# CliMA/ClimaSeaIce.jl

Measured on AMD Instinct MI355X. Metric: EVP sub-cycle cell-updates/s, higher is better.
Workload: dtype f64; 1 GPU; evp_subcycle_fplane_periodic_2048x2048_as_1x1_tiles_of_2048x2048_120substeps; substeps=120, mode=fast, halo=4, halo_exchange=none (one tile)

## Files before the change

climaseaice.jl_amd/csrc/evp_fast_math.h:

```cpp
#pragma once
#include "csi_dev.h"

namespace csi {
namespace fm {

#define CSI_EPS64 2.220446049250313e-16

__device__ __forceinline__ double fma_(double a, double b, double c) { return __builtin_fma(a, b, c); }
__device__ __forceinline__ double fmax_(double a, double b) { return __builtin_fmax(a, b); }
__device__ __forceinline__ double fmin_(double a, double b) { return __builtin_fmin(a, b); }
__device__ __forceinline__ double clampd(double x, double lo, double hi) { return x > hi ? hi : (x < lo ? lo : x); }
__device__ __forceinline__ double avg2(double a, double b) { return 0.5 * (a + b); }
__device__ __forceinline__ double avg4(double a, double b, double c, double d) { return 0.25 * ((a + b) + (c + d)); }
__device__ __forceinline__ double sum2(double a, double b) { return a + b; }
__device__ __forceinline__ double quarter(double s_a, double s_b) { return 0.25 * (s_a + s_b); }

__device__ __forceinline__ double rcp(double x) {
    const double r = __builtin_amdgcn_rcp(x);
    return fma_(fma_(-x, r, 1.0), r, r);
}
__device__ __forceinline__ double rsqrt(double x) {
    const double y = __builtin_amdgcn_rsq(x);
    const double g = x * y, h = 0.5 * y;
    const double r = fma_(-h, g, 0.5);
    return fma_(y, r, y);
}
__device__ __forceinline__ void sqrt_rsqrt(double x, double& s, double& rs) {
    const double y = __builtin_amdgcn_rsq(x);
    double g = x * y, h = 0.5 * y;
    const double r = fma_(-h, g, 0.5);
    g = fma_(g, r, g);
    h = fma_(h, r, h);
    const double d = fma_(-g, g, x);
    s = fma_(d, h, g);
    rs = 2.0 * h;
}
__device__ __forceinline__ double sqrt_fast(double x) {
    const double y = __builtin_amdgcn_rsq(x);
    const double g = x * y, h = 0.5 * y;
    const double r = fma_(-h, g, 0.5);
    return fma_(g, r, g);
}

template <bool UNI>
__device__ __forceinline__ void strain_cell(double A, double Bn, double Bs, double Cn, double Cs,
                                            double u_e, double u_w, double v_n, double v_s, double& e11, double& e22) {
    if (UNI) {
        e11 = A * (u_e - u_w);
        e22 = Cn * (v_n - v_s);
    } else {
        e11 = fma_(A, u_e - u_w, fma_(Bn, v_n, -(Bs * v_s)));
        e22 = fma_(Cn, v_n, -(Cs * v_s));
    }
}
template <bool UNI>
__device__ __forceinline__ double strain_corner(double Sn, double Ss, double Sv, double u_n, double u_s, double v_e, double v_w) {
    if (UNI) return fma_(Sv, v_e - v_w, Sn * (u_n - u_s));
    return fma_(Sv, v_e - v_w, fma_(Sn, u_n, -(Ss * u_s)));
}

struct StressConst {
    double em2, Dmin, Dmin2, rDmin, amin, amax, amin2, amax2, ramin, ramax;
    double hk1;
    int pressure_kind;
    double em2_8, Dmin2_16;
};

struct StressOut {
    double s11, s22, s12, alpha, zc2, zf2;
    double xc, rDc;
};

__device__ __forceinline__ StressOut stress_update_r(const StressConst& k, double e11c, double e22c, double e12f,
                                                     double e11f, double e22f, double e12c, double Pc, double Pf,
                                                     double mc, double mf, double rmc, double rmf, double hkc, double hkf,
                                                     double s11, double s22, double s12) {
    StressOut o;
    const double dc = e11c + e22c, df = e11f + e22f;
    const double tc = e11c - e22c, tf = e11f - e22f;
    const double sc2 = fma_(tc, tc, 4.0 * (e12c * e12c));
    const double sf2 = fma_(tf, tf, 4.0 * (e12f * e12f));
    const double xc = fmax_(fma_(dc, dc, sc2 * k.em2), k.Dmin2), xf = fmax_(fma_(df, df, sf2 * k.em2), k.Dmin2);
    const double rDc = rsqrt(xc), rDf = rsqrt(xf);
    const double zc2 = Pc * rDc, zf2 = Pf * rDf;
    const double Pr = (k.pressure_kind == 0) ? Pc * rcp(fma_(k.Dmin, rDc, 1.0)) : Pc;
    const double ec2 = zc2 * k.em2, ef2 = zf2 * k.em2;
    const double bulk = fma_(zc2 * k.hk1, dc, -0.5 * Pr);
    const double s11n = fma_(ec2, e11c, bulk);
    const double s22n = fma_(ec2, e22c, bulk);
    const double s12n = ef2 * e12f;
    const double g2c_raw = zc2 * hkc * rmc, g2f_raw = zf2 * hkf * rmf;
    const double g2c = fmax_(fmin_(g2c_raw, k.amax2), k.amin2);
    const double g2f = fmax_(fmin_(g2f_raw, k.amax2), k.amin2);
    double gc, rgc, gf, rgf;
    sqrt_rsqrt(g2c, gc, rgc);
    sqrt_rsqrt(g2f, gf, rgf);
    const double wc = (mc > 0) ? rgc : 0.0, wf = (mf > 0) ? rgf : 0.0;
    o.s11 = fma_(s11n - s11, wc, s11);
    o.s22 = fma_(s22n - s22, wc, s22);
    o.s12 = fma_(s12n - s12, wf, s12);
    o.alpha = gc;
    o.zc2 = zc2; o.zf2 = zf2; o.xc = xc; o.rDc = rDc;
    return o;
}

__device__ __forceinline__ StressOut stress_update_s(const StressConst& k, double e11c, double e22c, double E12f,
                                                     double S11f, double S22f, double y2, double Pc, double XP,
                                                     double mc, double M4, double rmc, double rM4, double hkc, double hkf4,
                                                     double s11, double s22, double s12) {
    StressOut o;
    const double dc = e11c + e22c, DF = S11f + S22f;
    const double tc = e11c - e22c, TF = S11f - S22f;
    const double sc2 = fma_(tc, tc, y2 * y2);
    const double sf2 = fma_(TF, TF, E12f * E12f);
    const double xc = fmax_(fma_(dc, dc, sc2 * k.em2), k.Dmin2), xf = fmax_(fma_(DF, DF, sf2 * k.em2), k.Dmin2_16);
    const double rDc = rsqrt(xc), rDf = rsqrt(xf);
    const double zc2 = Pc * rDc, zf2 = XP * rDf;
    const double Pr = (k.pressure_kind == 0) ? Pc * rcp(fma_(k.Dmin, rDc, 1.0)) : Pc;
    const double ec2 = zc2 * k.em2, ef2 = zf2 * k.em2_8;
    const double bulk = fma_(zc2 * k.hk1, dc, -0.5 * Pr);
    const double s11n = fma_(ec2, e11c, bulk);
    const double s22n = fma_(ec2, e22c, bulk);
    const double s12n = ef2 * E12f;
    const double g2c_raw = zc2 * hkc * rmc, g2f_raw = zf2 * hkf4 * rM4;
    const double g2c = fmax_(fmin_(g2c_raw, k.amax2), k.amin2);
    const double g2f = fmax_(fmin_(g2f_raw, k.amax2), k.amin2);
    double gc, rgc, gf, rgf;
    sqrt_rsqrt(g2c, gc, rgc);
    sqrt_rsqrt(g2f, gf, rgf);
    const double wc = (mc > 0) ? rgc : 0.0, wf = (M4 > 0) ? rgf : 0.0;
    o.s11 = fma_(s11n - s11, wc, s11);
    o.s22 = fma_(s22n - s22, wc, s22);
    o.s12 = fma_(s12n - s12, wf, s12);
    o.alpha = gc;
    o.zc2 = zc2; o.zf2 = zf2; o.xc = xc; o.rDc = rDc;
    return o;
}

__device__ __forceinline__ StressOut stress_update(const StressConst& k, double e11c, double e22c, double e12f,
                                                   double e11f, double e22f, double e12c, double Pc, double Pf,
                                                   double mc, double mf, double hkc, double hkf,
                                                   double s11, double s22, double s12) {
    return stress_update_r(k, e11c, e22c, e12f, e11f, e22f, e12c, Pc, Pf, mc, mf, rcp(mc), rcp(mf), hkc, hkf, s11, s22, s12);
}

struct VelConst {
    double dt, rdt, fcor, min_mass, min_conc;
    int has_cor;
};

__device__ __forceinline__ void ext_stress(int kind, double tau, double rhoCd, double we, double webar, double w, double wbar,
                                           double& ex, double& im) {
    if (kind == 3) {
        const double d1 = we - w, d2 = webar - wbar;
        const double n2 = fma_(d1, d1, d2 * d2);
        const double n = sqrt_fast(fmax_(n2, 2.2250738585072014e-308));
        im = rhoCd * n;
        ex = im * we;
    } else {
        ex = tau; im = 0.0;
    }
}

__device__ __forceinline__ void ext_stress_rest(double rhoCd, double w, double wbar, double& ex, double& im) {
    const double n2 = fma_(w, w, wbar * wbar);
    im = rhoCd * sqrt_fast(fmax_(n2, 2.2250738585072014e-308));
    ex = 0.0;
}

__device__ __forceinline__ double vel_update_avg(const VelConst& k, double w, double wn, double mi, double ai, double abar,
                                                 double div, double cor, double ext, double imt, double exb, double imb, bool peripheral) {
    const double rm = rcp(mi);
    const double rai = rm * ai;
    const double G = fma_(wn - w, k.rdt, fma_(div, rm, fma_(exb - ext, rai, cor)));
    const double tau_i = (imb - imt) * rai;
    const double wD = fma_(k.dt, G, abar * w) * rcp(fma_(k.dt, tau_i, abar));
    const bool active_ice = (mi >= k.min_mass) & (ai >= k.min_conc);
    double res = active_ice ? wD : 0.0;
    return peripheral ? 0.0 : res;
}
__device__ __forceinline__ double vel_update_avg_fd(const VelConst& k, double w, double wn, double mi, double ai, double abar,
                                                    double div, double cor, double ext, double imt, double exb, double imb,
                                                    bool peripheral, double wf) {
    const double wD = vel_update_avg(k, w, wn, mi, ai, abar, div, cor, ext, imt, exb, imb, false);
    const bool active_ice = (mi >= k.min_mass) & (ai >= k.min_conc);
    const bool marginal = (mi > CSI_EPS64) & (ai > CSI_EPS64);
    const double res = active_ice ? wD : (marginal ? wf : 0.0);
    return peripheral ? 0.0 : res;
}
__device__ __forceinline__ double vel_update(const VelConst& k, double w, double wn, double m_a, double m_b, double a_a, double a_b,
                                             double al_a, double al_b, double div, double cor,
                                             double ext, double imt, double exb, double imb, bool peripheral) {
    return vel_update_avg(k, w, wn, avg2(m_a, m_b), avg2(a_a, a_b), avg2(al_a, al_b), div, cor, ext, imt, exb, imb, peripheral);
}
__device__ __forceinline__ double vel_update_fd(const VelConst& k, double w, double wn, double m_a, double m_b, double a_a, double a_b,
                                                double al_a, double al_b, double div, double cor,
                                                double ext, double imt, double exb, double imb, bool peripheral, double wf) {
    return vel_update_avg_fd(k, w, wn, avg2(m_a, m_b), avg2(a_a, a_b), avg2(al_a, al_b), div, cor, ext, imt, exb, imb, peripheral, wf);
}

__device__ __forceinline__ double vel_update_sum(const VelConst& k2, double w, double wn, double m2, double a2, double al2,
                                                 double div2, double cor, double ext, double imt, double exb, double imb, bool peripheral) {
    const double rm2 = rcp(m2);
    const double rai = rm2 * a2;
    const double G = fma_(wn - w, k2.rdt, fma_(div2, rm2, fma_(exb - ext, rai, cor)));
    const double tau_i = (imb - imt) * rai;
    const double wD = fma_(k2.dt, G, al2 * w) * rcp(fma_(k2.dt, tau_i, al2));
    const bool active_ice = (m2 >= k2.min_mass) & (a2 >= k2.min_conc);
    double res = active_ice ? wD : 0.0;
    return peripheral ? 0.0 : res;
}
__device__ __forceinline__ double vel_update_sum_fd(const VelConst& k2, double w, double wn, double m2, double a2, double al2,
                                                    double div2, double cor, double ext, double imt, double exb, double imb,
                                                    bool peripheral, double wf) {
    const double wD = vel_update_sum(k2, w, wn, m2, a2, al2, div2, cor, ext, imt, exb, imb, false);
    const bool active_ice = (m2 >= k2.min_mass) & (a2 >= k2.min_conc);
    const bool marginal = (m2 > 2.0 * CSI_EPS64) & (a2 > 2.0 * CSI_EPS64);
    const double res = active_ice ? wD : (marginal ? wf : 0.0);
    return peripheral ? 0.0 : res;
}

__device__ __forceinline__ double div1(double E, double Fn, double Fs, double s11_0, double s11_m, double s12_p, double s12_0) {
    return fma_(E, s11_0 - s11_m, fma_(Fn, s12_p, -(Fs * s12_0)));
}
template <bool UNI>
__device__ __forceinline__ double div2(double Q1n, double Q2n, double Q1s, double Q2s, double K,
                                       double s11_0, double s22_0, double s11_m, double s22_m, double s12_p, double s12_0) {
    if (UNI) return fma_(K, s12_p - s12_0, Q2n * (s22_0 - s22_m));
    const double n = fma_(Q1n, s11_0, Q2n * s22_0);
    const double s = fma_(Q1s, s11_m, Q2s * s22_m);
    return fma_(K, s12_p - s12_0, n - s);
}

__device__ __forceinline__ void full_strain_cell(double Uy_e, double Uy_w, double Vx_n, double Vx_s, double Ur_e, double Ur_w,
                                                 double Vr_n, double Vr_s, double dyc2, double dxc2, double razc, double& e11, double& e22) {
    const double D1 = (Uy_e - Uy_w) + (Vx_n - Vx_s);
    const double D2 = fma_(dyc2, Ur_e - Ur_w, -(dxc2 * (Vr_n - Vr_s)));
    const double hr = 0.5 * razc;
    e11 = hr * (D1 + D2);
    e22 = hr * (D1 - D2);
}
__device__ __forceinline__ double full_strain_corner(double Ux_n, double Ux_s, double Vy_e, double Vy_w, double dxf2, double dyf2, double razf) {
    return (0.5 * razf) * fma_(dxf2, Ux_n - Ux_s, dyf2 * (Vy_e - Vy_w));
}
__device__ __forceinline__ double full_div1(double dyu, double rdyu, double rdxu, double razu, double S_e, double S_w, double T_e, double T_w,
                                            double Z_n, double Z_s) {
    return razu * fma_(0.5 * dyu, S_e - S_w, fma_(0.5 * rdyu, T_e - T_w, rdxu * (Z_n - Z_s)));
}
__device__ __forceinline__ double full_div2(double dxv, double rdxv, double rdyv, double razv, double S_n, double S_s, double T_n, double T_s,
                                            double Z_e, double Z_w) {
    return razv * fma_(0.5 * dxv, S_n - S_s, fma_(-0.5 * rdxv, T_n - T_s, rdyv * (Z_e - Z_w)));
}

__device__ __forceinline__ double full_strain_corner8(double Ux_n, double Ux_s, double Vy_e, double Vy_w, double dxf2, double dyf2, double razf) {
    return (4.0 * razf) * fma_(dxf2, Ux_n - Ux_s, dyf2 * (Vy_e - Vy_w));
}
__device__ __forceinline__ double full_div1_x2(double dyu, double rdyu, double rdxu, double razu, double S_e, double S_w, double T_e, double T_w,
                                               double Z_n, double Z_s) {
    return razu * fma_(dyu, S_e - S_w, fma_(rdyu, T_e - T_w, (rdxu + rdxu) * (Z_n - Z_s)));
}
__device__ __forceinline__ double full_div2_x2(double dxv, double rdxv, double rdyv, double razv, double S_n, double S_s, double T_n, double T_s,
                                               double Z_e, double Z_w) {
    return razv * fma_(dxv, S_n - S_s, fma_(-rdxv, T_n - T_s, (rdyv + rdyv) * (Z_e - Z_w)));
}

}
}
```

climaseaice.jl_amd/csrc/evp_fused2.hip:

```cpp
#include "evp_pair_stage.h"

#include <cstdio>
#include <cstdlib>

#ifndef CSI_PAIR_WAVES
#define CSI_PAIR_WAVES 3
#endif
#ifndef CSI_PAIR_UNI_WAVES
#define CSI_PAIR_UNI_WAVES 2
#endif
#ifndef CSI_PAIR_FULL_WAVES
#define CSI_PAIR_FULL_WAVES 2
#endif
#ifndef CSI_PAIR_PRIO
#define CSI_PAIR_PRIO 2
#endif
#ifndef CSI_PAIR_HOIST
#define CSI_PAIR_HOIST 1
#endif
#ifndef CSI_FULL_FENCE
#define CSI_FULL_FENCE 1
#endif
#ifndef CSI_PAIR_STORES
#define CSI_PAIR_STORES 7
#endif
#ifndef CSI_PEER_EXP
#define CSI_PEER_EXP 3
#endif
#ifndef CSI_PAIR_SKIPB
#define CSI_PAIR_SKIPB 0
#endif
#ifndef CSI_PAIR_PD
#define CSI_PAIR_PD 1
#endif

namespace csi {
namespace fused {

#ifdef CSI_PAIR_PROBE
static __device__ unsigned long long g_probe[8192 * 16];
#define PROBE_DECL unsigned long long pacc0 = 0, pacc1 = 0, pacc2 = 0, ptprev = 0, pit = 0; const unsigned long long pwall0 = wall_clock64()
#define PROBE_START do { __builtin_amdgcn_sched_barrier(0); ptprev = __builtin_readcyclecounter(); __builtin_amdgcn_sched_barrier(0); ++pit; } while (0)
#define PROBE(acc) do { __builtin_amdgcn_sched_barrier(0); const unsigned long long t_ = __builtin_readcyclecounter(); \
                        __builtin_amdgcn_sched_barrier(0); acc += t_ - ptprev; ptprev = t_; } while (0)
#define PROBE_END(slot) do { if (lane == 0 && (slot) < 8192 && !write_diag) { unsigned long long* dbg = g_probe + (size_t)(slot) * 16; \
                        dbg[0] = pacc0; dbg[1] = pacc1; dbg[2] = pacc2; dbg[6] = pit; dbg[8] = pwall0; dbg[9] = wall_clock64(); \
                        dbg[12] = PSTAGE.sp0; dbg[13] = PSTAGE.sp1; dbg[14] = PSTAGE.sp2; dbg[15] = PSTAGE.sp3; \
                        dbg[10] = (unsigned long long)__builtin_amdgcn_s_getreg((31 << 11) | (0 << 6) | 4); dbg[11] = (unsigned long long)blockIdx.x; } } while (0)
#else
#define PROBE_DECL do { } while (0)
#define PROBE_START do { } while (0)
#define PROBE(acc) do { } while (0)
#define PROBE_END(slot) do { } while (0)
#endif

template <int V> struct Idx { static constexpr int value = V; };

constexpr int RING_ROWS = 4;
enum : int { RF_S11 = 0, RF_S22, RF_S12, RF_U, RF_V, RF_P, RF_M, RF_A, RF_UN, RF_VN, RF_PF, RF_RMC, RF_RMF };
#ifndef CSI_PAIR_LDSC_NOPRE
#define CSI_PAIR_LDSC_NOPRE 1
#endif
#ifndef CSI_PAIR_PRE
#define CSI_PAIR_PRE 1
#endif
#ifndef CSI_PAIR_FRING
#define CSI_PAIR_FRING 1
#endif
constexpr int RF_FORCING = 8;
enum : int { RF_FU_TAU = 10, RF_FU_WE, RF_FU_WB, RF_FU_FD, RF_FV_TAU, RF_FV_WE, RF_FV_WB, RF_FV_FD };
constexpr int RP_ROWS = 3, RP_FIELDS = 12;
enum : int { RP_DXV = 0, RP_RDYV, RP_RDXU, RP_DXF2, RP_DYF2, RP_RAZF, RP_DYU, RP_DYC2, RP_DXC2, RP_RAZC, RP_RAZU, RP_RAZV };

template <bool UNI, bool AUF, bool WALLS, bool MASK, bool FORCE, bool FD, int CF, bool FULL = false, bool PEER = false, int EXTRA = 0, bool DLD = false>
__device__ __forceinline__ void pair_body(const FusedTable* __restrict__ table, const int w, int nstrips, int nchunks, int rows,
                                       int blocks_per_xcd, int write_diag, unsigned long long seq,
                                       double* __restrict__ ring, unsigned* __restrict__ ringm, double* __restrict__ outr, unsigned* __restrict__ peer_abort_p, double* __restrict__ ringp,
                                       double* __restrict__ ringc) {
    constexpr bool LDSC = !UNI && !FULL && !(EXTRA == 1 && MASK) && (CSI_PAIR_LDSC != 0);
    constexpr bool FRING = FORCE && !FULL && (EXTRA != 1 || !MASK) && CSI_PAIR_FRING;
    constexpr bool PRE = CSI_PAIR_PRE && !MASK && !FULL && !FRING && !(CSI_PAIR_LDSC_NOPRE && !UNI && !(EXTRA == 1 && MASK) && (CSI_PAIR_LDSC != 0));
    constexpr int RING_FIELDS = FRING ? 10 + RF_FORCING : (PRE ? 13 : 10);
#define peer_abort (*peer_abort_p)
    const int b = (int)blockIdx.x;
#ifndef CSI_EXP_ROLESWAP
#define CSI_EXP_ROLESWAP 0
#endif
    const bool consumer = (__builtin_amdgcn_readfirstlane((int)(threadIdx.x >> 6)) != 0) != (CSI_EXP_ROLESWAP && ((((b >> 3) / CSI_EXP_ROLESWAP) & 1) != 0));
    const int chunk = w / nstrips, strip = w - chunk * nstrips;
    const int lane = (int)(threadIdx.x & 63);
    tptr_t T = (tptr_t)table;
    const bool single = (write_diag & 2) != 0;
    write_diag &= 1;

    int ja, jb, rstart, rend;
    unsigned loff, sc, sf;
    unsigned lm = 0, sm = 0;
    int i;
    unsigned flags;
    int dx;
    int dxv;
    bool wave_valx_b = false;
    bool wave_has_dx_b;
    bool lanes_uniform;
    bool lanes_same;
    int row0;
    enum : unsigned { L_RS = 1, L_R1 = 2, L_R2 = 4, L_WALL_U = 8, L_WALL_V = 16, L_MIR_LO = 32, L_MIR_HI = 64, L_VAL_LO = 128, L_VAL_HI = 256, L_LOW = 512 };
    {
        const int Nx = T->I[FI_NX], Hx = T->I[FI_HX], Hy = T->I[FI_HY];
        const int i0s = T->I[FI_DEC + 0] - P_LO + strip * P_W;
        i = i0s + lane;
        {
            const int elo = T->I[FI_ELO] > 0 ? T->I[FI_ELO] : rows;
            ja = (T->I[FI_EHI] > 0 && chunk == nchunks - 1 && chunk > 0) ? T->I[FI_DEC + 3] - T->I[FI_EHI] + 1
                                                                         : T->I[FI_DEC + 2] + (chunk == 0 ? 0 : elo + (chunk - 1) * rows);
            jb = chunk == 0 ? min(ja + elo - 1, T->I[FI_DEC + 3])
                            : (chunk == nchunks - 1 ? T->I[FI_DEC + 3] : min(ja + rows - 1, T->I[FI_DEC + 3] - T->I[FI_EHI]));
        }
        const int ic = min(max(i, 1 - Hx), Nx + Hx);
        loff = (unsigned)(ic - (1 - Hx)) * 8u;
        row0 = 1 - Hy;
        const bool own = (lane >= P_LO) & (lane <= P_HI) & (i <= T->I[FI_DEC + 1]);
        flags = 0;
        if (own & (i >= T->I[FI_RS + 0]) & (i <= T->I[FI_RS + 1])) flags |= L_RS;
        if (own & (i >= T->I[FI_R1 + 0]) & (i <= T->I[FI_R1 + 1])) flags |= L_R1;
        if (own & (i >= T->I[FI_R2 + 0]) & (i <= T->I[FI_R2 + 1])) flags |= L_R2;
        dx = 0;
        if ((T->I[FI_XLO] == SIDE_PERIODIC) & (i >= 1) & (i <= Hx)) dx = Nx * 8;
        else if ((T->I[FI_XHI] == SIDE_PERIODIC) & (i > Nx - Hx) & (i <= Nx)) dx = -Nx * 8;
        dxv = dx;
        if (WALLS) {
            const bool xlo_wall = T->I[FI_XLO] == SIDE_WALL, xhi_wall = T->I[FI_XHI] == SIDE_WALL;
            if ((xlo_wall & (i <= 1)) | (xhi_wall & (i > Nx))) flags |= L_WALL_U;
            if ((xlo_wall & (i < 1)) | (xhi_wall & (i > Nx))) flags |= L_WALL_V;
            if (xlo_wall & (i == 0)) flags |= L_MIR_LO;
            if (xhi_wall & (i == Nx + 1)) flags |= L_MIR_HI;
            const bool vval_lo = T->I[FI_IMV + 0] == IMG_VALUE, vval_hi = T->I[FI_IMV + 1] == IMG_VALUE;
            if (xlo_wall & (i >= 1) & (i <= Hx)) dxv = vval_lo ? ((i == 1) ? -8 : 0) : (1 - 2 * i) * 8;
            if (xhi_wall & (i > Nx - Hx) & (i <= Nx)) dxv = vval_hi ? ((i == Nx) ? 8 : 0) : (2 * Nx + 1 - 2 * i) * 8;
            if (xlo_wall & vval_lo & ((i == 1) | (i == 0))) flags |= L_VAL_LO;
            if (xhi_wall & vval_hi & ((i == Nx) | (i == Nx + 1))) flags |= L_VAL_HI;
            wave_valx_b = __builtin_amdgcn_ballot_w64((flags & (L_VAL_LO | L_VAL_HI)) != 0) != 0;
        }
        wave_has_dx_b = __builtin_amdgcn_ballot_w64((dx != 0) | (dxv != 0)) != 0;
        const bool same = ((flags & L_RS) != 0) == ((flags & L_R1) != 0) && ((flags & L_RS) != 0) == ((flags & L_R2) != 0);
        lanes_same = __builtin_amdgcn_ballot_w64(!same) == 0;
        lanes_uniform = !wave_has_dx_b && lanes_same;
        rstart = max(ja - 3, T->I[FI_AJ0]);
#ifndef CSI_EXP_RINGCUT
#define CSI_EXP_RINGCUT 0
#endif
        rend = min(jb + 3 - CSI_EXP_RINGCUT, T->I[FI_AJ1]);
        if (i <= Hx) flags |= L_LOW;
        sc = (unsigned)T->I[FI_LD_C] * 8u;
        sf = (unsigned)T->I[FI_LD_F] * 8u;
        if (MASK) {
            sm = (unsigned)T->I[FI_MASK_LD];
            lm = (unsigned)(ic - (1 - Hx));
        }
    }
    unsigned pdirs = 0;
    if constexpr (PEER) {
        const bool pw = strip < T->I[FI_PSET], pe = strip >= nstrips - T->I[FI_PSET + 1], ps = chunk < T->I[FI_PSET + 2],
                   pn = chunk >= nchunks - T->I[FI_PSET + 3];
        pdirs = ((pw ? 1u : 0u) | (pe ? 2u : 0u) | (ps ? 4u : 0u) | (pn ? 8u : 0u) | ((ps & pw) ? 16u : 0u) | ((ps & pe) ? 32u : 0u) |
                 ((pn & pw) ? 64u : 0u) | ((pn & pe) ? 128u : 0u)) & (unsigned)T->I[FI_PMASK];
        pdirs = (unsigned)__builtin_amdgcn_readfirstlane((int)pdirs);
        if (pdirs) {
            if (!consumer && !(CSI_PEER_EXP & 4)) {
                const unsigned long long t0 = wall_clock64();
                bool dead = false;
                for (;;) {
                    bool behind = false, poison = false;
                    if constexpr ((CSI_PEER_EXP & 8) != 0) {
                        const unsigned long long* slots = (const unsigned long long*)T->P[FP_SLOT_IN + 2];
                        if (lane < 15) {
                            const int cq = (chunk + lane / 3 - 2 + 2 * nchunks) % nchunks, cs = (strip + lane % 3 - 1 + nstrips) % nstrips;
                            behind |= __hip_atomic_load(slots + (cq * nstrips + cs), __ATOMIC_RELAXED, __HIP_MEMORY_SCOPE_SYSTEM) + 1ull < seq;
                        }
                    } else
#pragma unroll
                    for (int d = 0; d < 8; ++d) {
                        if (!((pdirs >> d) & 1u)) continue;
                        const int nslots = T->I[FI_PWAIT + d];
                        const unsigned long long* slots = (const unsigned long long*)T->P[FP_SLOT_IN + d];
#pragma unroll 1
                        for (int b0 = 0; b0 < nslots; b0 += 64) {
                            const int idx = b0 + lane;
                            if (idx < nslots) behind |= __hip_atomic_load(slots + idx, __ATOMIC_RELAXED, __HIP_MEMORY_SCOPE_SYSTEM) + 1ull < seq;
                        }
                        if (lane == 63) poison |= __hip_atomic_load(slots + (kPeerSlots - 1), __ATOMIC_RELAXED, __HIP_MEMORY_SCOPE_SYSTEM) != 0ull;
                    }
                    if (__builtin_amdgcn_ballot_w64(behind) == 0) break;
                    if (__builtin_amdgcn_ballot_w64(poison | (*(volatile unsigned*)T->P[FP_PERR] != 0u)) != 0 || wall_clock64() - t0 > 300000000ull) { dead = true; break; }
                    __builtin_amdgcn_s_sleep(8);
                }
                if (dead) {
                    if (lane == 0) *(volatile unsigned*)T->P[FP_PERR] = 1u;
                    if (lane < 8) {
                        typedef const __attribute__((address_space(4))) unsigned long* sptr_t;
                        unsigned long long* out = (unsigned long long*)((sptr_t)&T->P[FP_SLOT_OUT])[lane];
                        if (out) __hip_atomic_store(out + (kPeerSlots - 1), 1ull, __ATOMIC_RELAXED, __HIP_MEMORY_SCOPE_SYSTEM);
                    }
                }
                if (lane == 0) peer_abort = dead ? 1u : 0u;
                if (T->I[FI_PTIER] >= 1) __builtin_amdgcn_fence(__ATOMIC_ACQUIRE, "");
                __builtin_amdgcn_sched_barrier(0);
            }
            __syncthreads();
            if (peer_abort) return;
        }
    }
    auto offc = [&](int j) __attribute__((always_inline)) { return loff + (unsigned)(j - row0) * sc; };
    auto offf = [&](int j) __attribute__((always_inline)) { return loff + (unsigned)(j - row0) * sf; };
    auto offm = [&](int j) __attribute__((always_inline)) { return lm + (unsigned)(j - row0) * sm; };
    const int NyW = T->I[FI_NY], HyW = T->I[FI_HY];
    int rcd = 0;
    if constexpr (FULL) {
        typedef const __attribute__((address_space(4))) int* iptr_t;
        iptr_t rcs = (iptr_t)T->P[FP_RCSUM];
        if (rcs) {
            const int t0 = max(rstart - 4, row0) - row0, t1 = min(rend + 2, NyW + HyW + 1) - row0;
            if (rcs[t1 + 1] - rcs[t0] == t1 - t0 + 1) rcd = FP_C2ROW_0 - FP_C2_0;
        }
    }
    const unsigned c2s = FULL ? (rcd ? 8u : (unsigned)T->I[FI_C2_LD] * 8u) : 0u;
    const unsigned loff2 = (FULL && rcd) ? 0u : loff;
    auto off2 = [&](int j) __attribute__((always_inline)) { return loff2 + (unsigned)(j - row0) * c2s; };
    const int NyLoW = PEER ? T->I[FI_NYLO] : NyW;
    const bool wrap_lo_b = T->I[FI_YLO] == SIDE_PERIODIC, wrap_hi_b = T->I[FI_YHI] == SIDE_PERIODIC;
    const bool ylo_wall_b = WALLS && T->I[FI_YLO] == SIDE_WALL, yhi_wall_b = WALLS && T->I[FI_YHI] == SIDE_WALL;
    const bool uval_lo_b = WALLS && T->I[FI_IMU + 2] == IMG_VALUE, uval_hi_b = WALLS && T->I[FI_IMU + 3] == IMG_VALUE;
    enum : unsigned { U_WRAPLO = 1, U_YLO = 2, U_YHI = 4, U_UVLO = 8, U_UVHI = 16, U_HASDX = 32, U_VALX = 64, U_WRAPHI = 128, U_MIR = 256 };
    const bool wave_mir_b = WALLS && __builtin_amdgcn_ballot_w64((flags & (L_MIR_LO | L_MIR_HI)) != 0) != 0;
    const unsigned UF = (unsigned)__builtin_amdgcn_readfirstlane((int)((wrap_lo_b ? U_WRAPLO : 0u) | (wrap_hi_b ? U_WRAPHI : 0u) | (ylo_wall_b ? U_YLO : 0u) | (yhi_wall_b ? U_YHI : 0u) |
                                                                         (uval_lo_b ? U_UVLO : 0u) | (uval_hi_b ? U_UVHI : 0u) |
                                                                         (wave_has_dx_b ? U_HASDX : 0u) | (wave_valx_b ? U_VALX : 0u) | (wave_mir_b ? U_MIR : 0u)));
#define wrap_lo ((UF & U_WRAPLO) != 0)
#define wrap_hi ((UF & U_WRAPHI) != 0)
#define ylo_wall (WALLS && (UF & U_YLO) != 0)
#define yhi_wall (WALLS && (UF & U_YHI) != 0)
#define uval_lo (WALLS && (UF & U_UVLO) != 0)
#define uval_hi (WALLS && (UF & U_UVHI) != 0)
#define wave_has_dx ((UF & U_HASDX) != 0)
#define wave_valx (WALLS && (UF & U_VALX) != 0)
#define wave_mir (WALLS && (UF & U_MIR) != 0)
#define has_dld (PEER && DLD)
    auto wall_row = [&](int j) __attribute__((always_inline)) { return (ylo_wall & (j < 1)) | (yhi_wall & (j > NyW)); };
    auto wall_vrow = [&](int j) __attribute__((always_inline)) { return (ylo_wall & (j <= 1)) | (yhi_wall & (j > NyW)); };
    const bool lane_wu = WALLS && (flags & L_WALL_U) != 0, lane_wv = WALLS && (flags & L_WALL_V) != 0;
    auto numbers = [&](Forcing& F) __attribute__((always_inline)) {
        F.t_tau_u = T->K[FK_TOP_TAU_U]; F.t_we_u = T->K[FK_TOP_UE]; F.t_wb_u = T->K[FK_TOP_VE];
        F.b_tau_u = T->K[FK_BOT_TAU_U]; F.b_we_u = T->K[FK_BOT_UE]; F.b_wb_u = T->K[FK_BOT_VE];
        F.t_tau_v = T->K[FK_TOP_TAU_V]; F.t_we_v = T->K[FK_TOP_VE]; F.t_wb_v = T->K[FK_TOP_UE];
        F.b_tau_v = T->K[FK_BOT_TAU_V]; F.b_we_v = T->K[FK_BOT_VE]; F.b_wb_v = T->K[FK_BOT_UE];
        F.fd_u = 0.0; F.fd_v = 0.0; F.fd = FD;
        F.xc_u = 0.0; F.xd_u = 0.0; F.xc_v = 0.0; F.xd_v = 0.0; F.extra = EXTRA == 1 ? T->I[FI_EXTRA] : 0;
    };
    auto arrays = [&](Forcing& F, unsigned ou, unsigned ov) __attribute__((always_inline)) {
        if (T->I[FI_TOP_KIND] == 2) { F.t_tau_u = ldg(T->P[FP_FT_U], ou); F.t_tau_v = ldg(T->P[FP_FT_V], ov); }
        if constexpr (EXTRA == 2) {
            if (T->I[FI_TOP_UEK] == 2) { F.t_we_u = ldg(T->P[FP_FT_U], ou); F.t_wb_v = ldg(T->P[FP_FT_UBAR], ov); }
            if (T->I[FI_TOP_VEK] == 2) { F.t_we_v = ldg(T->P[FP_FT_V], ov); F.t_wb_u = ldg(T->P[FP_FT_VBAR], ou); }
            if (T->I[FI_BOT_KIND] == 2) { F.b_tau_u = ldg(T->P[FP_FB_U], ou); F.b_tau_v = ldg(T->P[FP_FB_V], ov); }
        }
        if (T->I[FI_BOT_UEK] == 2) { F.b_we_u = ldg(T->P[FP_FB_U], ou); F.b_wb_v = ldg(T->P[FP_FB_UBAR], ov); }
        if (T->I[FI_BOT_VEK] == 2) { F.b_we_v = ldg(T->P[FP_FB_V], ov); F.b_wb_u = ldg(T->P[FP_FB_VBAR], ou); }
        if (FD) { F.fd_u = ldg(T->P[FP_FD_U], ou); F.fd_v = ldg(T->P[FP_FD_V], ov); }
        if (EXTRA == 1) {
            if (F.extra & 1) { F.xc_u = ldg(T->P[FP_XC_U], ou); F.xc_v = ldg(T->P[FP_XC_V], ov); }
            if (F.extra & 2) { F.xd_u = ldg(T->P[FP_XD_U], ou); F.xd_v = ldg(T->P[FP_XD_V], ov); }
        }
    };
    auto stress_consts = [&](fm::StressConst& ks) __attribute__((always_inline)) {
        ks.em2 = T->K[FK_EM2]; ks.Dmin = T->K[FK_DMIN]; ks.Dmin2 = T->K[FK_DMIN2]; ks.rDmin = T->K[FK_RDMIN];
        ks.amin = T->K[FK_AMIN]; ks.amax = T->K[FK_AMAX]; ks.amin2 = T->K[FK_AMIN2]; ks.amax2 = T->K[FK_AMAX2];
        ks.ramin = T->K[FK_RAMIN]; ks.ramax = T->K[FK_RAMAX]; ks.hk1 = T->K[FK_HK1]; ks.pressure_kind = T->I[FI_PRESSURE_KIND];
        ks.em2_8 = T->K[FK_PK_EM2_8]; ks.Dmin2_16 = T->K[FK_PK_DMIN2_16];
    };
    auto vel_consts = [&](fm::VelConst& kv) __attribute__((always_inline)) {
        kv.dt = T->K[FK_DT2]; kv.rdt = T->K[FK_RDT]; kv.fcor = T->K[FK_FCOR]; kv.min_mass = T->K[FK_MIN_MASS2];
        kv.min_conc = T->K[FK_MIN_CONC2]; kv.has_cor = T->I[FI_HAS_COR];
    };
    const int prio_rank = (int)(__builtin_amdgcn_s_getreg((3 << 11) | (0 << 6) | 4) % 3u);
    auto set_prio = [&](int k) __attribute__((always_inline)) {
        if (CSI_PAIR_PRIO == 2) {
            if (consumer) __builtin_amdgcn_s_setprio(2); else __builtin_amdgcn_s_setprio(0);
        } else if (CSI_PAIR_PRIO == 3) {
            if (consumer) __builtin_amdgcn_s_setprio(0); else __builtin_amdgcn_s_setprio(2);
        } else if (CSI_PAIR_PRIO == 4) {
            if (consumer) __builtin_amdgcn_s_setprio(3); else __builtin_amdgcn_s_setprio(0);
        } else if (CSI_PAIR_PRIO) {
            int p = prio_rank + k;
            p = p >= 3 ? p - 3 : p;
            if (p == 0) __builtin_amdgcn_s_setprio(0); else if (p == 1) __builtin_amdgcn_s_setprio(1); else __builtin_amdgcn_s_setprio(2);
        }
    };
    const int rs_lo = max(ja, T->I[FI_RS + 2]), rs_hi = min(jb, T->I[FI_RS + 3]);
    const int r1_lo = max(ja, T->I[FI_R1 + 2]), r1_hi = min(jb, T->I[FI_R1 + 3]);
    const int r2_lo = max(ja, T->I[FI_R2 + 2]), r2_hi = min(jb, T->I[FI_R2 + 3]);
    auto yimg = [&](int j) __attribute__((always_inline)) {
        return (wrap_lo & (j >= 1) & (j <= HyW)) ? NyLoW : ((wrap_hi & (j > NyW - HyW) & (j <= NyW)) ? -NyW : 0);
    };
    auto yimg_u = [&](int j) __attribute__((always_inline)) {
        int d = yimg(j);
        if (WALLS) {
            if (ylo_wall & (j >= 1) & (j <= HyW)) d = uval_lo ? ((j == 1) ? -1 : 0) : 1 - 2 * j;
            if (yhi_wall & (j > NyW - HyW) & (j <= NyW)) d = uval_hi ? ((j == NyW) ? 1 : 0) : 2 * NyW + 1 - 2 * j;
        }
        return d;
    };
    enum : int { D_W = 0, D_E, D_S, D_N, D_SW, D_SE, D_NW, D_NE };
    auto own = [&](int k) __attribute__((always_inline)) { return T->P[k < 5 ? FP_S11_OUT + k : FP_AL + (k - 5)]; };
    auto img = [&](int k, int d) __attribute__((always_inline)) { return PEER ? T->P[FP_IMG0 + d * 9 + k] : own(k); };
    const bool wave_low = PEER && __builtin_amdgcn_ballot_w64(((flags & L_LOW) != 0) & ((dx != 0) | (dxv != 0))) != 0;
    const bool wt = T->I[FI_WT] != 0;
    auto sto = [&](unsigned long b_, unsigned o_, double v_) __attribute__((always_inline)) {
        if (wt) stg_agent(b_, o_, v_); else stg(b_, o_, v_);
    };
    auto put4 = [&](int k, unsigned off, unsigned dy, bool ylow, int dxl, double val, double valy, double valx, double valxy, int j, int yr) __attribute__((always_inline)) {
        const unsigned long base = own(k);
        auto sti = [&](unsigned long b_, unsigned o_, double v_) __attribute__((always_inline)) {
            if constexpr (PEER && (CSI_PEER_EXP & 2) != 0)
                __scoped_atomic_store_n((__attribute__((address_space(1))) long*)((gptr_t)b_ + o_), __builtin_bit_cast(long, v_), __ATOMIC_RELAXED, __MEMORY_SCOPE_SYSTEM);
            else sto(b_, o_, v_);
        };
        sto(base, off, val);
        if constexpr (PEER) {
            if (has_dld) {
                const int cls = (k == 2 || k == 3 || k == 7) ? 1 : 0;
                const int p0 = j + HyW - 1, p1 = p0 + yr;
                const int dY = ylow ? D_S : D_N, dX = wave_low ? D_W : D_E;
                const int dXY = ylow ? (wave_low ? D_SW : D_SE) : (wave_low ? D_NW : D_NE);
                if (dy != 0u) sti(img(k, dY), off + dy + (unsigned)(p1 * T->I[FI_PDLD + dY * 2 + cls]), valy);
                if (wave_has_dx && dxl != 0) {
                    sti(img(k, dX), off + (unsigned)dxl + (unsigned)(p0 * T->I[FI_PDLD + dX * 2 + cls]), valx);
                    if (dy != 0u) sti(img(k, dXY), off + (unsigned)dxl + dy + (unsigned)(p1 * T->I[FI_PDLD + dXY * 2 + cls]), valxy);
                }
                return;
            }
        }
        if (dy != 0u) sti(PEER ? (ylow ? img(k, D_S) : img(k, D_N)) : base, off + dy, valy);
        if (wave_has_dx) {
            if (dxl != 0) {
                sti(PEER ? (wave_low ? img(k, D_W) : img(k, D_E)) : base, off + (unsigned)dxl, valx);
                if (dy != 0u) sti(PEER ? (ylow ? (wave_low ? img(k, D_SW) : img(k, D_SE)) : (wave_low ? img(k, D_NW) : img(k, D_NE))) : base, off + (unsigned)dxl + dy, valxy);
            }
        }
    };
    auto put = [&](int k, unsigned off, unsigned dy, bool ylow, int dxl, double val, int j, int yr) __attribute__((always_inline)) {
        put4(k, off, dy, ylow, dxl, val, val, val, val, j, yr);
    };
    auto put_u = [&](unsigned off, int j, unsigned dy, double val, int yr) __attribute__((always_inline)) {
        double vy = val;
        if (WALLS) {
            if (uval_lo & ylo_wall & (j == 1)) vy = 2 * T->K[FK_BCU] - val;
            if (uval_hi & yhi_wall & (j == NyW)) vy = 2 * T->K[FK_BCU + 1] - val;
        }
        put4(3, off, dy, j <= HyW, dx, val, vy, val, vy, j, yr);
    };
    auto put_v = [&](unsigned off, unsigned dy, bool ylow, double val, int j, int yr) __attribute__((always_inline)) {
        double vx = val;
        if (WALLS && wave_valx) {
            if (flags & L_VAL_LO) vx = 2 * T->K[FK_BCV] - val;
            if (flags & L_VAL_HI) vx = 2 * T->K[FK_BCV + 1] - val;
        }
        put4(4, off, dy, ylow, dxv, val, val, vx, vx, j, yr);
    };
    int fast_lo, fast_hi;
    {
        const int d1 = AUF ? 0 : 1;
        fast_lo = max(rs_lo, max(r1_lo + d1, r2_lo + 1));
        fast_hi = min(rs_hi, min(r1_hi + d1, r2_hi + 1));
        if (wrap_lo | ylo_wall) fast_lo = max(fast_lo, HyW + 2);
        if (wrap_hi | yhi_wall) fast_hi = min(fast_hi, NyW - HyW);
    }
    const bool fast_plain = lanes_uniform;
    auto flush = [&](int q, double v11, double v22, double v12, double vfirst, double vsecond, auto WH, auto VFT) __attribute__((always_inline)) {
        constexpr int which = decltype(WH)::value;
        constexpr bool VF = decltype(VFT)::value != 0;
        if (which == 0) return;
        if ((q >= fast_lo) & (q <= fast_hi)) {
            const unsigned ocq = offc(q), ofq = offf(q);
            if (fast_plain) {
                if (flags & L_RS) {
                    if (which & 1) { sto(T->P[FP_S11_OUT], ocq, v11); sto(T->P[FP_S22_OUT], ocq, v22); sto(T->P[FP_S12_OUT], ofq, v12); }
                    if (which & 2) sto(T->P[VF ? FP_V_OUTP : FP_U_OUTP], VF ? ocq : ofq - sf, vfirst);
                    if (which & 4) sto(T->P[VF ? FP_U_OUTP : FP_V_OUTP], VF ? ofq - sf : ocq - sc, vsecond);
                }
            } else {
                const bool ls = (flags & L_RS) != 0, l1 = (flags & L_R1) != 0, l2 = (flags & L_R2) != 0;
                if ((which & 1) && ls) { put(0, ocq, 0u, false, dx, v11, q, 0); put(1, ocq, 0u, false, dx, v22, q, 0); put(2, ofq, 0u, false, dx, v12, q, 0); }
                if (VF) { if ((which & 2) && l1) put_v(ocq, 0u, false, vfirst, q, 0); if ((which & 4) && l2) put(3, ofq - sf, 0u, false, dx, vsecond, q - 1, 0); }
                else { if ((which & 2) && l1) put(3, ofq - sf, 0u, false, dx, vfirst, q - 1, 0); if ((which & 4) && l2) put_v(ocq - sc, 0u, false, vsecond, q - 1, 0); }
            }
            return;
        }
        const int j1 = VF ? q : q - 1, j2 = q - 1;
        const bool do_s = ((which & 1) != 0) & (q >= rs_lo) & (q <= rs_hi), do_1 = ((which & 2) != 0) & (j1 >= r1_lo) & (j1 <= r1_hi),
                   do_2 = ((which & 4) != 0) & (j2 >= r2_lo) & (j2 <= r2_hi);
        if (!(do_s | do_1 | do_2)) return;
        const unsigned ocq = offc(q), ofq = offf(q);
        const unsigned o1 = VF ? ocq : ofq - sf;
        const unsigned o2 = VF ? ofq - sf : ocq - sc;
        const int yq = yimg(q), y1 = VF ? yimg(j1) : yimg_u(j1), y2 = VF ? yimg_u(j2) : yimg(j2);
        if (do_s & ((flags & L_RS) != 0)) {
            put(0, ocq, (unsigned)yq * sc, q <= HyW, dx, v11, q, yq);
            put(1, ocq, (unsigned)yq * sc, q <= HyW, dx, v22, q, yq);
            put(2, ofq, (unsigned)yq * sf, q <= HyW, dx, v12, q, yq);
        }
        if (do_1 & ((flags & L_R1) != 0)) {
            if (VF) put_v(o1, (unsigned)y1 * sc, j1 <= HyW, vfirst, j1, y1); else put_u(o1, j1, (unsigned)y1 * sf, vfirst, y1);
        }
        if (do_2 & ((flags & L_R2) != 0)) {
            if (VF) put_u(o2, j2, (unsigned)y2 * sf, vsecond, y2); else put_v(o2, (unsigned)y2 * sc, j2 <= HyW, vsecond, j2, y2);
        }
    };
    unsigned lane_it = (unsigned)lane;
    auto fresh_lane = [&]() __attribute__((always_inline)) {
        if constexpr (MASK && !FULL) {
            unsigned l;
            asm volatile("v_mbcnt_lo_u32_b32 %0, -1, 0\n\tv_mbcnt_hi_u32_b32 %0, -1, %0" : "=v"(l));
            lane_it = l;
        }
    };
    auto rslot = [&](int j) __attribute__((always_inline)) { return (unsigned)((j - rstart) & (RING_ROWS - 1)) * (RING_FIELDS * 64) + lane_it; };

#ifndef CSI_PAIR_UNROLL
#define CSI_PAIR_UNROLL 3
#endif

    if (!consumer) {
        PROBE_DECL;
        Stage<UNI, AUF, MASK, FORCE, CF, FULL, !(EXTRA == 1 && MASK)> A;
        A.lc = ringc;
        const int cjmin = LDSC ? T->I[FI_COEF_JMIN] : 0, cjmax = LDSC ? T->I[FI_COEF_JMAX] : 0;
        const unsigned ck_lane = (unsigned)min(lane, FC_COUNT - 1) * 8u;
        auto coef_row_base = [&](int j) __attribute__((always_inline)) {
            return T->P[FP_PCOEF_VEC] + (unsigned long)((long)min(max(j, cjmin), cjmax) * (long)(FC_COUNT * 8));
        };
#ifndef CSI_EXP_RINGALIAS
#define CSI_EXP_RINGALIAS 0
#endif
        auto alias_row = [&](int j) __attribute__((always_inline)) { return CSI_EXP_RINGALIAS ? min(max(j, ja + 1), max(jb - 1, ja + 1)) : j; };
        unsigned oc = offc(alias_row(rstart)), of = offf(alias_row(rstart)), om = MASK ? offm(rstart) : 0u;
        {
            const double rho0 = T->K[FK_RHO];
            A.u_m = ldg(T->P[FP_U_IN], of - sf); A.v_m = ldg(T->P[FP_V_IN], oc - sc);
            A.u_0 = ldg(T->P[FP_U_IN], of); A.v_0 = ldg(T->P[FP_V_IN], oc);
            A.a_mm = 0.0; A.a_m = ldg(T->P[FP_A], oc - sc);
            A.m_mm = 0.0; A.m_m = ldg(T->P[FP_H], oc - sc) * rho0 * A.a_m;
            const double P_m = ldg(T->P[FP_P], oc - sc);
            A.XP_m = fm::sum2(from_left(P_m), P_m);
            A.Xm_m = fm::sum2(from_left(A.m_m), A.m_m);
            A.Xa_m = fm::sum2(from_left(A.a_m), A.a_m);
            A.Xv_m = fm::sum2(from_left(A.v_m), A.v_m);
            A.Xv_0 = fm::sum2(from_left(A.v_0), A.v_0);
            double e11_m, e22_m;
            const int jm = rstart - 1;
            A.hoist_uniform(T);
            if constexpr (FULL) {
                const unsigned om2 = off2(jm), o02 = off2(rstart);
                full_cell(T, om2, c2s, A.u_m, A.v_m, A.v_0, e11_m, e22_m, rcd);
                A.e12_0 = 8.0 * full_corner(T, o02, c2s, A.u_0, A.u_m, A.v_0, rcd);
                A.hoist_planes(T, rcd);
                A.full_init(T, o02, om2, c2s);
            } else {
            fm::strain_cell<UNI>(pcoef<UNI>(T, FC_A, jm), pcoef<UNI>(T, FC_BN, jm), pcoef<UNI>(T, FC_BS, jm), pcoef<UNI>(T, FC_CN, jm),
                            pcoef<UNI>(T, FC_CS, jm), from_right(A.u_m), A.u_m, A.v_0, A.v_m, e11_m, e22_m);
            A.e12_0 = fm::strain_corner<UNI>(pcoef<UNI>(T, FC_SN, rstart), pcoef<UNI>(T, FC_SS, rstart), pcoef<UNI>(T, FC_SV, rstart), A.u_0, A.u_m, A.v_0, from_left(A.v_0));
            }
            A.Xe11_m = fm::sum2(from_left(e11_m), e11_m);
            A.Xe22_m = fm::sum2(from_left(e22_m), e22_m);
            A.Ye12_0 = fm::sum2(A.e12_0, from_right(A.e12_0));
            A.XAL_m = 0; A.XS11L_m = 0; A.XS22L_m = 0; A.XW = 0; A.Wprev = 0;
            A.S11_mm = 0; A.S22_mm = 0; A.S12_mm = 0; A.AL_mm = 0; A.S11_m = 0; A.S22_m = 0; A.S12_m = 0; A.AL_m = 0;
            A.S11_0 = 0; A.S22_0 = 0; A.S12_0 = 0; A.AL_0 = 0; A.first = 0; A.second = 0;
        }
#pragma unroll
        for (int q = 0; q < RING_ROWS * RING_FIELDS; ++q) ring[q * 64 + lane] = 0.0;
        if constexpr (FULL) {
#pragma unroll
            for (int q = 0; q < RP_ROWS * RP_FIELDS; ++q) ringp[q * 64 + lane] = 1.0;
            A.RAZU_m = 1.0; A.RAZV_x = 1.0; A.RAZC_0 = 1.0;
        }
        unsigned mhist = 0xffffffffu;
        if (MASK) {
            const bool wi = lane_wv | wall_row(rstart - 1);
            const unsigned act = ldub(T->P[FP_MASK], om - sm);
            mhist = (mhist << 2) | (wi ? 3u : (act ? 0u : 1u));
            ringm[(unsigned)((-1) & (RING_ROWS - 1)) * 64 + (unsigned)lane] = mhist & 3u;
        }
        RowIn R[3];
#ifndef CSI_FULL_HOISTP
#define CSI_FULL_HOISTP 1
#endif
#ifndef CSI_FORCE_HOIST
#define CSI_FORCE_HOIST 0
#endif
        constexpr bool HIN = (FULL && CSI_FULL_HOISTP >= 2) || (FORCE && !FULL && (CSI_FORCE_HOIST & 1));
        const unsigned long hU = HIN ? T->P[FP_U_IN] : 0ul, hV = HIN ? T->P[FP_V_IN] : 0ul, hP = HIN ? T->P[FP_P] : 0ul, hH = HIN ? T->P[FP_H] : 0ul,
                            hA = HIN ? T->P[FP_A] : 0ul, h11 = HIN ? T->P[FP_S11_IN] : 0ul, h22 = HIN ? T->P[FP_S22_IN] : 0ul, h12 = HIN ? T->P[FP_S12_IN] : 0ul,
                            hUN = HIN ? T->P[FP_UN] : 0ul, hVN = HIN ? T->P[FP_VN] : 0ul;
        int rnext = rstart;
        auto load_row = [&](RowIn& Q) __attribute__((always_inline)) {
            if constexpr (HIN) {
                Q.u_p = ldg(hU, of + sf); Q.v_p = ldg(hV, oc + sc);
                Q.P_0 = ldg(hP, oc); Q.h_0 = ldg(hH, oc); Q.a_0 = ldg(hA, oc);
                Q.s11 = ldg(h11, oc); Q.s22 = ldg(h22, oc); Q.s12 = ldg(h12, of);
                Q.un_m = ldg(hUN, of - sf); Q.vn_x = ldg(hVN, AUF ? oc - sc : oc);
            } else {
            Q.u_p = ldg(T->P[FP_U_IN], of + sf); Q.v_p = ldg(T->P[FP_V_IN], oc + sc);
            Q.P_0 = ldg(T->P[FP_P], oc); Q.h_0 = ldg(T->P[FP_H], oc); Q.a_0 = ldg(T->P[FP_A], oc);
            Q.s11 = ldg(T->P[FP_S11_IN], oc); Q.s22 = ldg(T->P[FP_S22_IN], oc); Q.s12 = ldg(T->P[FP_S12_IN], of);
            Q.un_m = ldg(T->P[FP_UN], of - sf); Q.vn_x = ldg(T->P[FP_VN], AUF ? oc - sc : oc);
            }
            Q.mk = MASK ? ldub(T->P[FP_MASK], om) : 1u;
            if constexpr (LDSC) Q.ck = ldg(coef_row_base(rnext + 2), ck_lane);
        };
        auto advance = [&]() __attribute__((always_inline)) {
            const bool more = rnext < rend;
            if (CSI_EXP_RINGALIAS) { rnext += more ? 1 : 0; oc = offc(alias_row(rnext)); of = offf(alias_row(rnext)); return; }
            oc += more ? sc : 0u; of += more ? sf : 0u;
            if (MASK) om += more ? sm : 0u;
            rnext += more ? 1 : 0;
        };
        int r = rstart;
        auto body = [&](auto KK) __attribute__((always_inline)) {
            constexpr int k = decltype(KK)::value;
            if (!CSI_PAIR_HOIST || FORCE || (FULL && CSI_FULL_FENCE)) asm volatile("" : "+s"(T));
            set_prio(k);
            fresh_lane();
            PROBE_START;
            if (CSI_PAIR_PD == 1) __builtin_amdgcn_s_waitcnt(0x0F70);
            else if (MASK) __builtin_amdgcn_s_waitcnt(0x0F70 | 11);
            else __builtin_amdgcn_s_waitcnt(0x0F70 | 10);
            PROBE(pacc0);
            const RowIn& C = R[k];
            if constexpr (LDSC) { if (lane < FC_COUNT) ringc[(unsigned)((r + 2) & 7) * FC_COUNT + (unsigned)lane] = C.ck; }
            const unsigned so = (unsigned)((r - rstart) & 1) * (5 * 64) + (unsigned)lane;
            constexpr int PW = 7 & ~CSI_PAIR_STORES;
            double o11 = 0, o22 = 0, o12 = 0, ofirst = 0, osecond = 0;
            if (PW & 1) { o11 = outr[so]; o22 = outr[so + 64]; o12 = outr[so + 128]; }
            if (PW & 2) ofirst = outr[so + 192];
            if (PW & 4) osecond = outr[so + 256];
            Forcing FA;
            numbers(FA);
            if (FORCE) arrays(FA, offf(r - 1), AUF ? offc(r - 1) : offc(r));
            if constexpr (!FULL) {
                advance();
                load_row(R[(k + CSI_PAIR_PD) % 3]);
            }
            flush(r - 4, o11, o22, o12, ofirst, osecond, Idx<PW>{}, Idx<AUF ? 1 : 0>{});
            fm::StressConst ks; stress_consts(ks);
            fm::VelConst kv; vel_consts(kv);
            const double m_0 = C.h_0 * T->K[FK_RHO] * C.a_0;
            const bool pa1 = WALLS && (AUF ? (lane_wu | wall_row(r - 1)) : (lane_wv | wall_vrow(r)));
            const bool pa2 = WALLS && (AUF ? (lane_wv | wall_vrow(r - 1)) : (lane_wu | wall_row(r - 1)));
            if (MASK) {
                const bool wi = lane_wv | wall_row(r);
                mhist = (mhist << 2) | (wi ? 3u : (C.mk ? 0u : 1u));
            }
            if constexpr (FULL) {
                static_assert(CSI_PAIR_PD == 1, "the per-point-metric producer prefetches one row ahead");
                auto mid = [&]() __attribute__((always_inline)) { advance(); load_row(R[(k + 1) % 3]); };
                A.template step<false>(T, ks, kv, r, C.u_p, C.v_p, C.P_0, m_0, C.a_0, C.s11, C.s22, C.s12, C.un_m, C.vn_x, true, r > rstart, pa1, pa2, mhist, FA,
                                       off2(r), c2s, off2(min(r + 1, rend)), off2(max(r - 1, row0)), mid);
            } else
            A.step(T, ks, kv, r, C.u_p, C.v_p, C.P_0, m_0, C.a_0, C.s11, C.s22, C.s12, C.un_m, C.vn_x, true, r > rstart, pa1, pa2, mhist, FA);
            {
                const unsigned s0 = rslot(r), s1 = rslot(r - 1);
                ring[s0 + RF_S11 * 64] = A.S11_0; ring[s0 + RF_S22 * 64] = A.S22_0; ring[s0 + RF_S12 * 64] = A.S12_0;
                if (AUF) { ring[s1 + RF_U * 64] = A.first; ring[s1 + RF_V * 64] = A.second; }
                else { ring[s0 + RF_V * 64] = A.first; ring[s1 + RF_U * 64] = A.second; }
                if (single) {
                    ring[s0 + RF_P * 64] = A.AL_0; ring[s0 + RF_M * 64] = 0.5 * A.zf; ring[s0 + RF_A * 64] = 0.5 * A.zc; ring[s0 + RF_VN * 64] = A.Dc * A.rDc;
                } else {
                ring[s0 + RF_P * 64] = C.P_0; ring[s0 + RF_M * 64] = m_0; ring[s0 + RF_A * 64] = C.a_0;
                if (PRE) { ring[s0 + RF_PF * 64] = A.Pf_0; ring[s0 + RF_RMC * 64] = A.rmc_0; ring[s0 + RF_RMF * 64] = A.rmf_0; }
                ring[s1 + RF_UN * 64] = C.un_m; ring[(AUF ? s1 : s0) + RF_VN * 64] = C.vn_x;
                }
                if constexpr (FRING) {
                    if constexpr (EXTRA == 2) {
                        const bool tt = T->I[FI_TOP_KIND] == 2, bt = T->I[FI_BOT_KIND] == 2;
                        ring[s0 + RF_FU_TAU * 64] = tt ? FA.t_tau_u : FA.t_we_u; ring[s0 + RF_FU_FD * 64] = FA.t_wb_u;
                        ring[s0 + RF_FU_WE * 64] = bt ? FA.b_tau_u : FA.b_we_u; ring[s0 + RF_FU_WB * 64] = FA.b_wb_u;
                        ring[s0 + RF_FV_TAU * 64] = tt ? FA.t_tau_v : FA.t_we_v; ring[s0 + RF_FV_FD * 64] = FA.t_wb_v;
                        ring[s0 + RF_FV_WE * 64] = bt ? FA.b_tau_v : FA.b_we_v; ring[s0 + RF_FV_WB * 64] = FA.b_wb_v;
                    } else {
                    ring[s0 + RF_FU_TAU * 64] = FA.t_tau_u; ring[s0 + RF_FU_WE * 64] = FA.b_we_u; ring[s0 + RF_FU_WB * 64] = FA.b_wb_u; ring[s0 + RF_FU_FD * 64] = EXTRA == 1 ? FA.xc_u : FA.fd_u;
                    ring[s0 + RF_FV_TAU * 64] = FA.t_tau_v; ring[s0 + RF_FV_WE * 64] = FA.b_we_v; ring[s0 + RF_FV_WB * 64] = FA.b_wb_v; ring[s0 + RF_FV_FD * 64] = EXTRA == 1 ? FA.xc_v : FA.fd_v;
                    }
                }
                if constexpr (FULL) {
                    const unsigned p0 = (unsigned)k * (RP_FIELDS * 64) + lane_it;
                    ringp[p0 + RP_DXV * 64] = A.DXV_p; ringp[p0 + RP_RDYV * 64] = A.RDYV_p; ringp[p0 + RP_RDXU * 64] = A.RDXU_p;
                    ringp[p0 + RP_DXF2 * 64] = A.DXF2_p; ringp[p0 + RP_DYF2 * 64] = A.DYF2_p; ringp[p0 + RP_RAZF * 64] = A.RAZF_p;
                    ringp[p0 + RP_DYU * 64] = A.DYU_0; ringp[p0 + RP_DYC2 * 64] = A.DYC2_0; ringp[p0 + RP_DXC2 * 64] = A.DXC2_0;
                    ringp[p0 + RP_RAZC * 64] = A.RAZC_0; ringp[p0 + RP_RAZU * 64] = A.RAZU_m; ringp[p0 + RP_RAZV * 64] = A.RAZV_x;
                }
                if (MASK) ringm[(unsigned)((r - rstart) & (RING_ROWS - 1)) * 64 + lane_it] = mhist & 3u;
            }
            A.shift(C.u_p, C.v_p, m_0, C.a_0);
            PROBE(pacc1);
#ifndef CSI_EXP_HALFBARRIER
#define CSI_EXP_HALFBARRIER 0
#endif
            if (!(CSI_EXP_HALFBARRIER && ((r - rstart) & 1)))
            __syncthreads();
            PROBE(pacc2);
        };
        if constexpr (LDSC) {
#pragma unroll
            for (int d = -3; d <= 1; ++d) {
                const double v = ldg(coef_row_base(rstart + d), ck_lane);
                if (lane < FC_COUNT) ringc[(unsigned)((rstart + d) & 7) * FC_COUNT + (unsigned)lane] = v;
            }
        }
        load_row(R[0]);
        if (CSI_PAIR_PD == 2) {
            advance();
            load_row(R[1]);
        }
        for (;;) {
            body(Idx<0>{});
            if (++r > rend) break;
            body(Idx<1>{});
            if (++r > rend) break;
            body(Idx<2>{});
            if (++r > rend) break;
        }
        for (int d = 0; d < 2; ++d) {
            const unsigned so = (unsigned)((r - rstart) & 1) * (5 * 64) + (unsigned)lane;
            flush(r - 4, outr[so], outr[so + 64], outr[so + 128], outr[so + 192], outr[so + 256], Idx<(7 & ~CSI_PAIR_STORES)>{}, Idx<AUF ? 1 : 0>{});
            if (d == 0) __syncthreads();
            ++r;
        }
#define PSTAGE A
        PROBE_END(w * 2);
#undef PSTAGE
        return;
    }

    auto publish = [&]() __attribute__((always_inline)) {
        if (PEER && pdirs) {
            if ((CSI_PEER_EXP & 1) && T->I[FI_PTIER] < 2) __builtin_amdgcn_s_waitcnt(0x0F70);
            else { __builtin_amdgcn_fence(__ATOMIC_RELEASE, ""); asm volatile("s_waitcnt vmcnt(0)" ::: "memory"); }
            if ((lane < 8) && ((pdirs >> lane) & 1u)) {
                const int nW = T->I[FI_PSET], nE = T->I[FI_PSET + 1], nN = T->I[FI_PSET + 3];
                const bool xw = (lane == D_W) | (lane == D_SW) | (lane == D_NW), xe = (lane == D_E) | (lane == D_SE) | (lane == D_NE);
                const bool yn = (lane == D_N) | (lane == D_NW) | (lane == D_NE);
                const int xs = xe ? strip - (nstrips - nE) : strip, xn = xw ? nW : (xe ? nE : nstrips);
                const int ys = yn ? chunk - (nchunks - nN) : chunk;
                typedef const __attribute__((address_space(4))) unsigned long* sptr_t;
                unsigned long long* out = (unsigned long long*)((sptr_t)&T->P[FP_SLOT_OUT])[lane];
                __hip_atomic_store(out + (ys * xn + xs), seq, __ATOMIC_RELAXED, __HIP_MEMORY_SCOPE_SYSTEM);
            }
        }
    };

    if (single) {
        {
            const int d1 = AUF ? 1 : 0;
            fast_lo = max(rs_lo, max(r1_lo + d1, r2_lo + 1));
            fast_hi = min(rs_hi, min(r1_hi + d1, r2_hi + 1));
            if (wrap_lo | ylo_wall) fast_lo = max(fast_lo, HyW + 2);
            if (wrap_hi | yhi_wall) fast_hi = min(fast_hi, NyW - HyW);
            }
        for (int r = rstart; r <= rend; ++r) {
            __syncthreads();
            const unsigned s0 = rslot(r), s1 = rslot(r - 1);
            const double v11 = ring[s0 + RF_S11 * 64], v22 = ring[s0 + RF_S22 * 64], v12 = ring[s0 + RF_S12 * 64];
            const double vfirst = AUF ? ring[s1 + RF_U * 64] : ring[s0 + RF_V * 64];
            const double vsecond = AUF ? ring[s1 + RF_V * 64] : ring[s1 + RF_U * 64];
            const double dal = ring[s0 + RF_P * 64], dzf = ring[s0 + RF_M * 64], dzc = ring[s0 + RF_A * 64], ddl = ring[s0 + RF_VN * 64];
            flush(r, v11, v22, v12, vfirst, vsecond, Idx<7>{}, Idx<AUF ? 0 : 1>{});
            if (write_diag) {
                if (((flags & L_RS) != 0) & (r >= rs_lo) & (r <= rs_hi)) {
                    const unsigned ocq = offc(r), ofq = offf(r);
                    const int yq = yimg(r);
                    put(5, ocq, (unsigned)yq * sc, r <= HyW, dx, dal, r, yq);
                    put(7, ofq, (unsigned)yq * sf, r <= HyW, dx, dzf, r, yq);
                    put(6, ocq, (unsigned)yq * sc, r <= HyW, dx, dzc, r, yq);
                    put(8, ocq, (unsigned)yq * sc, r <= HyW, dx, ddl, r, yq);
                }
            }
        }
        __syncthreads();
        publish();
        return;
    }

    PROBE_DECL;
    Stage<UNI, !AUF, MASK, FORCE, CF, FULL, !(EXTRA == 1 && MASK)> B;
    B.lc = ringc;
    B.u_m = 0; B.u_0 = 0; B.v_m = 0; B.v_0 = 0; B.Xv_m = 0; B.Xv_0 = 0;
    B.a_mm = 0; B.a_m = 0; B.m_mm = 0; B.m_m = 0;
    B.XP_m = 0; B.Xm_m = 0; B.Xa_m = 0; B.Xe11_m = 0; B.Xe22_m = 0; B.Ye12_0 = 0; B.e12_0 = 0;
    B.XAL_m = 0; B.XS11L_m = 0; B.XS22L_m = 0; B.XW = 0; B.Wprev = 0;
    B.S11_mm = 0; B.S22_mm = 0; B.S12_mm = 0; B.AL_mm = 0; B.S11_m = 0; B.S22_m = 0; B.S12_m = 0; B.AL_m = 0;
    B.S11_0 = 0; B.S22_0 = 0; B.S12_0 = 0; B.AL_0 = 0; B.first = 0; B.second = 0;
    B.zc = 0; B.zf = 0; B.Dc = 0; B.rDc = 0; B.Pf_0 = 0; B.rmc_0 = 0; B.rmf_0 = 0;
    B.hoist_uniform(T);
    if constexpr (FULL) {
        B.hoist_planes(T, rcd);
        B.full_init(T, off2(max(rstart - 2, row0)), off2(max(rstart - 3, row0)), c2s);
        B.full_prefetch_vel(T, off2(max(rstart - 2, row0)), off2(max(rstart - 3, row0)));
    }
    int fq = 0;
    bool fhave = false;
    double f11 = 0, f22 = 0, f12 = 0, ffirst = 0, fsecond = 0;
    const int rlo = rstart - 1;
    unsigned mhistB = 0xffffffffu;
    double vn_delay = 0.0;
    double razv_delay = 1.0;
    double fvd_tau = 0.0, fvd_we = 0.0, fvd_wb = 0.0, fvd_fd = 0.0;
    int r = rstart;
    auto bodyB = [&](auto KK) __attribute__((always_inline)) {
        if (!CSI_PAIR_HOIST || FORCE || (FULL && CSI_FULL_FENCE)) asm volatile("" : "+s"(T));
        set_prio(decltype(KK)::value);
        const int q = r - 2;
        PROBE_START;
        if (!(CSI_EXP_HALFBARRIER && ((r - rstart) & 1)))
        __syncthreads();
        PROBE(pacc0);
        if constexpr (!FULL && CSI_PAIR_SKIPB) { if (q < ja - 3) return; }
        fresh_lane();
        const unsigned s1 = rslot(r - 1), s2 = rslot(r - 2), s3 = rslot(r - 3);
        double bu_p = ring[s1 + RF_U * 64], bv_p = ring[s1 + RF_V * 64];
        const double s11 = ring[s2 + RF_S11 * 64], s22 = ring[s2 + RF_S22 * 64], s12 = ring[s2 + RF_S12 * 64];
        const double bP_0 = ring[s2 + RF_P * 64], bm_0 = ring[s2 + RF_M * 64], ba_0 = ring[s2 + RF_A * 64];
        if (PRE) { B.Pf_0 = ring[s2 + RF_PF * 64]; B.rmc_0 = ring[s2 + RF_RMC * 64]; B.rmf_0 = ring[s2 + RF_RMF * 64]; }
        const double bun = ring[s3 + RF_UN * 64], vn_new = ring[s2 + RF_VN * 64];
        const double bvn = AUF ? vn_new : vn_delay;
        vn_delay = vn_new;
        const unsigned bmk = MASK ? ringm[(unsigned)((r - 2 - rstart) & (RING_ROWS - 1)) * 64 + lane_it] : 0u;
        if constexpr (FULL) {
            if (fhave) flush(fq, f11, f22, f12, ffirst, fsecond, Idx<(CSI_PAIR_STORES & 7)>{}, Idx<AUF ? 1 : 0>{});
        }
        PROBE(pacc1);
        fm::StressConst ks; stress_consts(ks);
        fm::VelConst kv; vel_consts(kv);
        if (WALLS) {
            if (wave_mir) {
            const double vl = from_left(bv_p), vr = from_right(bv_p);
            double ml = vr, mh = vl;
            if (wave_valx) {
                if (flags & L_VAL_LO) ml = 2 * T->K[FK_BCV] - vr;
                if (flags & L_VAL_HI) mh = 2 * T->K[FK_BCV + 1] - vl;
            }
            bv_p = (flags & L_MIR_LO) ? ml : ((flags & L_MIR_HI) ? mh : bv_p);
            }
            if (ylo_wall & (q == 0)) B.u_0 = uval_lo ? 2 * T->K[FK_BCU] - bu_p : bu_p;
            if (yhi_wall & (q == NyW)) bu_p = uval_hi ? 2 * T->K[FK_BCU + 1] - B.u_0 : B.u_0;
        }
        if (MASK) mhistB = (mhistB << 2) | ((q >= rlo) ? bmk : 3u);
        Forcing FB;
        numbers(FB);
        if constexpr (FRING) {
            const double u0 = ring[s2 + RF_FU_TAU * 64], u1 = ring[s2 + RF_FU_WE * 64], u2 = ring[s2 + RF_FU_WB * 64], u3 = ring[s2 + RF_FU_FD * 64];
            double v0, v1, v2, v3;
            if (AUF) {
                v0 = ring[s1 + RF_FV_TAU * 64]; v1 = ring[s1 + RF_FV_WE * 64]; v2 = ring[s1 + RF_FV_WB * 64]; v3 = ring[s1 + RF_FV_FD * 64];
            } else {
                const double n0 = ring[s2 + RF_FV_TAU * 64], n1 = ring[s2 + RF_FV_WE * 64], n2 = ring[s2 + RF_FV_WB * 64], n3 = ring[s2 + RF_FV_FD * 64];
                v0 = fvd_tau; v1 = fvd_we; v2 = fvd_wb; v3 = fvd_fd;
                fvd_tau = n0; fvd_we = n1; fvd_wb = n2; fvd_fd = n3;
            }
            if constexpr (EXTRA == 2) {
                if (T->I[FI_TOP_KIND] == 2) { FB.t_tau_u = u0; FB.t_tau_v = v0; } else { FB.t_we_u = u0; FB.t_we_v = v0; }
                FB.t_wb_u = u3; FB.t_wb_v = v3;
                if (T->I[FI_BOT_KIND] == 2) { FB.b_tau_u = u1; FB.b_tau_v = v1; } else { FB.b_we_u = u1; FB.b_we_v = v1; }
                FB.b_wb_u = u2; FB.b_wb_v = v2;
            } else {
                FB.t_tau_u = u0; FB.b_we_u = u1; FB.b_wb_u = u2;
                FB.t_tau_v = v0; FB.b_we_v = v1; FB.b_wb_v = v2;
                if (EXTRA == 1) { FB.xc_u = u3; FB.xc_v = v3; } else { FB.fd_u = u3; FB.fd_v = v3; }
            }
        } else if (FORCE) {
            const int qm = max(q - 1, row0), qa = max(q, row0);
#ifndef CSI_EXP_NOCONSLOADS
            arrays(FB, offf(qm), AUF ? offc(qa) : offc(qm));
#endif
        }
        const bool pb1 = WALLS && (!AUF ? (lane_wu | wall_row(q - 1)) : (lane_wv | wall_vrow(q)));
        const bool pb2 = WALLS && (!AUF ? (lane_wv | wall_vrow(q - 1)) : (lane_wu | wall_row(q - 1)));
        if constexpr (FULL) {
            constexpr int kk = decltype(KK)::value;
            auto midB = [&]() __attribute__((always_inline)) {
                const unsigned pn = (unsigned)((kk + 2) % 3) * (RP_FIELDS * 64) + lane_it;
                B.N_DXV = ringp[pn + RP_DXV * 64]; B.N_RDYV = ringp[pn + RP_RDYV * 64]; B.N_RDXU = ringp[pn + RP_RDXU * 64];
                B.N_DXF2 = ringp[pn + RP_DXF2 * 64]; B.N_DYF2 = ringp[pn + RP_DYF2 * 64]; B.N_RAZF = ringp[pn + RP_RAZF * 64];
                B.N_DYU = ringp[pn + RP_DYU * 64]; B.N_DYC2 = ringp[pn + RP_DYC2 * 64]; B.N_DXC2 = ringp[pn + RP_DXC2 * 64];
                B.N_RAZC = ringp[pn + RP_RAZC * 64]; B.N_RAZU = ringp[pn + RP_RAZU * 64];
                if (AUF) B.N_RAZV = ringp[(unsigned)kk * (RP_FIELDS * 64) + lane_it + RP_RAZV * 64];
                else { const double x = ringp[pn + RP_RAZV * 64]; B.N_RAZV = razv_delay; razv_delay = x; }
            };
            B.template step<PRE, decltype(midB), true, true>(T, ks, kv, q, bu_p, bv_p, bP_0, bm_0, ba_0, s11, s22, s12, bun, bvn, q >= ja - 1, q >= ja, pb1, pb2, mhistB, FB,
                   off2(max(q, row0)), c2s, off2(max(q + 1, row0)), off2(max(q - 1, row0)), midB, off2(max(q, row0)));
            fq = q; f11 = B.S11_0; f22 = B.S22_0; f12 = B.S12_0; ffirst = B.first; fsecond = B.second; fhave = true;
        } else {
        B.template step<PRE>(T, ks, kv, q, bu_p, bv_p, bP_0, bm_0, ba_0, s11, s22, s12, bun, bvn, q >= ja - 1, q >= ja, pb1, pb2, mhistB, FB);
        flush(q, B.S11_0, B.S22_0, B.S12_0, B.first, B.second, Idx<(CSI_PAIR_STORES & 7)>{}, Idx<AUF ? 1 : 0>{});
        }
        if ((CSI_PAIR_STORES & 7) != 7) {
            const unsigned so = (unsigned)((r - rstart) & 1) * (5 * 64) + (unsigned)lane;
            if (!(CSI_PAIR_STORES & 1)) { outr[so] = B.S11_0; outr[so + 64] = B.S22_0; outr[so + 128] = B.S12_0; }
            if (!(CSI_PAIR_STORES & 2)) outr[so + 192] = B.first;
            if (!(CSI_PAIR_STORES & 4)) outr[so + 256] = B.second;
        }
        if (write_diag) {
            if (((flags & L_RS) != 0) & (q >= rs_lo) & (q <= rs_hi)) {
                const unsigned ocq = offc(q), ofq = offf(q);
                const int yq = yimg(q);
                put(5, ocq, (unsigned)yq * sc, q <= HyW, dx, B.AL_0, q, yq);
                put(7, ofq, (unsigned)yq * sf, q <= HyW, dx, 0.5 * B.zf, q, yq);
                put(6, ocq, (unsigned)yq * sc, q <= HyW, dx, 0.5 * B.zc, q, yq);
                put(8, ocq, (unsigned)yq * sc, q <= HyW, dx, B.Dc * B.rDc, q, yq);
            }
        }
        B.shift(bu_p, bv_p, bm_0, ba_0);
        PROBE(pacc2);
    };
    for (;;) {
        bodyB(Idx<0>{});
        if (++r > rend) break;
        bodyB(Idx<1>{});
        if (++r > rend) break;
        bodyB(Idx<2>{});
        if (++r > rend) break;
    }
    if constexpr (FULL) {
        if (fhave) flush(fq, f11, f22, f12, ffirst, fsecond, Idx<(CSI_PAIR_STORES & 7)>{}, Idx<AUF ? 1 : 0>{});
    }
    __syncthreads();
    publish();
#define PSTAGE B
    PROBE_END(w * 2 + 1);
#undef PSTAGE
#undef peer_abort
}

template <bool UNI, bool AUF, bool WALLS, bool MASK, bool FORCE, bool FD, int CF, bool FULL = false, bool PEER = false, int EXTRA = 0, bool DLD = false>
__global__ void __launch_bounds__(128, (FULL || (FORCE && (EXTRA != 1 || !MASK) && CSI_PAIR_FRING)) ? CSI_PAIR_FULL_WAVES
                                       : (UNI && !(EXTRA == 1 && MASK)) ? CSI_PAIR_UNI_WAVES : CSI_PAIR_WAVES) k_pair(const FusedTable* __restrict__ table, int nstrips, int nchunks, int rows,
                                                              int blocks_per_xcd, int write_diag, unsigned long long seq) {
    constexpr bool FRING = FORCE && !FULL && (EXTRA != 1 || !MASK) && CSI_PAIR_FRING;
    constexpr bool PRE = CSI_PAIR_PRE && !MASK && !FULL && !FRING && !(CSI_PAIR_LDSC_NOPRE && !UNI && !(EXTRA == 1 && MASK) && (CSI_PAIR_LDSC != 0));
    constexpr int RING_FIELDS = FRING ? 10 + RF_FORCING : (PRE ? 13 : 10);
    __shared__ double ring[RING_ROWS * RING_FIELDS * 64];
    __shared__ double ringp[FULL ? RP_ROWS * RP_FIELDS * 64 : 1];
    __shared__ unsigned ringm[MASK ? RING_ROWS * 64 : 1];
    __shared__ double outr[(CSI_PAIR_STORES & 7) != 7 ? 2 * 5 * 64 : 1];
    __shared__ unsigned peer_abort_w;
#ifdef CSI_EXP_LDSPAD
    __shared__ double lds_pad[(FULL && FORCE) ? CSI_EXP_LDSPAD / 8 : 1];
    if (FULL && FORCE) { lds_pad[threadIdx.x] = 0.0; asm volatile("" :: "v"(lds_pad[threadIdx.x])); }
#endif
    constexpr bool LDSC = !UNI && !FULL && !(EXTRA == 1 && MASK) && (CSI_PAIR_LDSC != 0);
    __shared__ double ringc[LDSC ? 8 * FC_COUNT : 1];
    const int b = (int)blockIdx.x;
    int w = (b & 7) * blocks_per_xcd + (b >> 3);
    if (write_diag & 12) {
        typedef const __attribute__((address_space(4))) int* iptr_t;
        iptr_t act = (iptr_t)((tptr_t)table)->P[(write_diag & 8) ? FP_ACT_LIVE0 : FP_ACT_LIVE];
        const int live = act[0], per = (live + 7) >> 3, k = b >> 3, p = (b & 7) * per + k;
        if ((k >= per) | (p >= live)) return;
        w = act[2 + p];
    } else if (w >= nstrips * nchunks) return;
    if constexpr (PEER) {
        const int chunk = w / nstrips, strip = w - chunk * nstrips;
        tptr_t T = (tptr_t)table;
        const bool pw = strip < T->I[FI_PSET], pe = strip >= nstrips - T->I[FI_PSET + 1], ps = chunk < T->I[FI_PSET + 2],
                   pn = chunk >= nchunks - T->I[FI_PSET + 3];
        const unsigned pd = ((pw ? 1u : 0u) | (pe ? 2u : 0u) | (ps ? 4u : 0u) | (pn ? 8u : 0u) | ((ps & pw) ? 16u : 0u) | ((ps & pe) ? 32u : 0u) |
                             ((pn & pw) ? 64u : 0u) | ((pn & pe) ? 128u : 0u)) & (unsigned)T->I[FI_PMASK];
        if (__builtin_amdgcn_readfirstlane((int)pd) == 0) {
            pair_body<UNI, AUF, WALLS, MASK, FORCE, FD, CF, FULL, false, EXTRA, false>(table, w, nstrips, nchunks, rows, blocks_per_xcd, write_diag, seq, ring, ringm, outr, &peer_abort_w, ringp, ringc);
            return;
        }
    }
    pair_body<UNI, AUF, WALLS, MASK, FORCE, FD, CF, FULL, PEER, EXTRA, DLD>(table, w, nstrips, nchunks, rows, blocks_per_xcd, write_diag, seq, ring, ringm, outr, &peer_abort_w, ringp, ringc);
}

}

#if defined(CSI_PAIR_PROBE) && (!defined(CSI_PAIR_VARIANT) || CSI_PAIR_VARIANT == 0)
extern "C" int csi_debug_probe(unsigned long long* dst) {
    return (int)hipMemcpyFromSymbol(dst, HIP_SYMBOL(fused::g_probe), sizeof(unsigned long long) * 8192 * 16);
}
#endif
#if defined(CSI_PAIR_PROBE) && defined(CSI_PAIR_VARIANT) && CSI_PAIR_VARIANT >= 1
#define CSI_PROBE_NAME_(v) csi_debug_probe_v##v
#define CSI_PROBE_NAME(v) CSI_PROBE_NAME_(v)
extern "C" int CSI_PROBE_NAME(CSI_PAIR_VARIANT)(unsigned long long* dst) {
    return (int)hipMemcpyFromSymbol(dst, HIP_SYMBOL(fused::g_probe), sizeof(unsigned long long) * 8192 * 16);
}
#endif

#ifndef CSI_PAIR_VARIANT
#define CSI_PAIR_VARIANT 0
#endif
#if CSI_PAIR_VARIANT == 0
#define CSI_PAIR_NAME launch_fused_pair_plain
#define CSI_PAIR_FLAGS false, false, false, false
#elif CSI_PAIR_VARIANT == 1
#define CSI_PAIR_NAME launch_fused_pair_walls
#define CSI_PAIR_FLAGS true, false, false, false
#elif CSI_PAIR_VARIANT == 2
#define CSI_PAIR_NAME launch_fused_pair_mask
#define CSI_PAIR_FLAGS true, true, false, false
#elif CSI_PAIR_VARIANT == 3
#define CSI_PAIR_NAME launch_fused_pair_force
#define CSI_PAIR_FLAGS true, false, true, false
#elif CSI_PAIR_VARIANT == 4
#define CSI_PAIR_NAME launch_fused_pair_mask_force
#define CSI_PAIR_FLAGS true, true, true, false
#elif CSI_PAIR_VARIANT == 5
#define CSI_PAIR_NAME launch_fused_pair_force_fd
#define CSI_PAIR_FLAGS true, false, true, true
#elif CSI_PAIR_VARIANT == 6
#define CSI_PAIR_NAME launch_fused_pair_mask_force_fd
#define CSI_PAIR_FLAGS true, true, true, true
#elif CSI_PAIR_VARIANT == 7
#define CSI_PAIR_NAME launch_fused_pair_force_x
#define CSI_PAIR_FLAGS true, false, true, false
#define CSI_PAIR_EXTRA 1
#elif CSI_PAIR_VARIANT == 8
#define CSI_PAIR_NAME launch_fused_pair_mask_force_x
#define CSI_PAIR_FLAGS true, true, true, false
#define CSI_PAIR_EXTRA 1
#elif CSI_PAIR_VARIANT == 9
#define CSI_PAIR_NAME launch_fused_pair_force_w
#define CSI_PAIR_FLAGS true, false, true, false
#define CSI_PAIR_EXTRA 2
#else
#define CSI_PAIR_NAME launch_fused_pair_mask_force_w
#define CSI_PAIR_FLAGS true, true, true, false
#define CSI_PAIR_EXTRA 2
#endif
#ifndef CSI_PAIR_EXTRA
#define CSI_PAIR_EXTRA 0
#endif
void CSI_PAIR_NAME(const FusedTable* dev_table, int metric, bool a_ufirst, int common, int nstrips, int nchunks, int rows,
                   int write_diag, unsigned long long seq, hipStream_t s) {
    const int nblocks = nstrips * nchunks;
    const int per_xcd = (nblocks + 7) / 8;
    dim3 grid((unsigned)(per_xcd * 8)), block(128);
    const bool dld = (seq >> 63) != 0;
    seq &= ~(1ull << 63);
    (void)dld;
#if CSI_PAIR_VARIANT >= 1
#define CSI_LAUNCH_PAIR_(U, A, C, F) do { if (seq && dld) hipLaunchKernelGGL((fused::k_pair<U, A, CSI_PAIR_FLAGS, C, F, true, CSI_PAIR_EXTRA, true>), grid, block, 0, s, dev_table, nstrips, nchunks, rows, per_xcd, write_diag, seq); \
                                          else if (seq) hipLaunchKernelGGL((fused::k_pair<U, A, CSI_PAIR_FLAGS, C, F, true, CSI_PAIR_EXTRA>), grid, block, 0, s, dev_table, nstrips, nchunks, rows, per_xcd, write_diag, seq); \
                                          else hipLaunchKernelGGL((fused::k_pair<U, A, CSI_PAIR_FLAGS, C, F, false, CSI_PAIR_EXTRA>), grid, block, 0, s, dev_table, nstrips, nchunks, rows, per_xcd, write_diag, seq); } while (0)
#else
#define CSI_LAUNCH_PAIR_(U, A, C, F) do { if (seq) hipLaunchKernelGGL((fused::k_pair<U, A, CSI_PAIR_FLAGS, C, F, true, CSI_PAIR_EXTRA>), grid, block, 0, s, dev_table, nstrips, nchunks, rows, per_xcd, write_diag, seq); \
                                          else hipLaunchKernelGGL((fused::k_pair<U, A, CSI_PAIR_FLAGS, C, F, false, CSI_PAIR_EXTRA>), grid, block, 0, s, dev_table, nstrips, nchunks, rows, per_xcd, write_diag, seq); } while (0)
#endif
#if CSI_PAIR_VARIANT <= 2
#define CSI_LAUNCH_PAIR(U, A) do { if (common == 2) CSI_LAUNCH_PAIR_(U, A, 2, false); else if (common) CSI_LAUNCH_PAIR_(U, A, 1, false); else CSI_LAUNCH_PAIR_(U, A, 0, false); } while (0)
#else
#define CSI_LAUNCH_PAIR(U, A) do { (void)common; CSI_LAUNCH_PAIR_(U, A, 0, false); } while (0)
#endif
    if (metric == 2) {
#if CSI_PAIR_VARIANT >= 1 && CSI_PAIR_VARIANT <= 2
        if (common == 2) { if (a_ufirst) CSI_LAUNCH_PAIR_(false, true, 2, true); else CSI_LAUNCH_PAIR_(false, false, 2, true); }
        else { if (a_ufirst) CSI_LAUNCH_PAIR_(false, true, 0, true); else CSI_LAUNCH_PAIR_(false, false, 0, true); }
#elif CSI_PAIR_VARIANT >= 1
        if (a_ufirst) CSI_LAUNCH_PAIR_(false, true, 0, true); else CSI_LAUNCH_PAIR_(false, false, 0, true);
#endif
    } else if (metric == 0) { if (a_ufirst) CSI_LAUNCH_PAIR(true, true); else CSI_LAUNCH_PAIR(true, false); }
    else { if (a_ufirst) CSI_LAUNCH_PAIR(false, true); else CSI_LAUNCH_PAIR(false, false); }
#undef CSI_LAUNCH_PAIR
#undef CSI_LAUNCH_PAIR_
}

#if CSI_PAIR_VARIANT == 0
void launch_fused_pair_walls(const FusedTable*, int, bool, int, int, int, int, int, unsigned long long, hipStream_t);
void launch_fused_pair_mask(const FusedTable*, int, bool, int, int, int, int, int, unsigned long long, hipStream_t);
void launch_fused_pair_force(const FusedTable*, int, bool, int, int, int, int, int, unsigned long long, hipStream_t);
void launch_fused_pair_mask_force(const FusedTable*, int, bool, int, int, int, int, int, unsigned long long, hipStream_t);
void launch_fused_pair_force_fd(const FusedTable*, int, bool, int, int, int, int, int, unsigned long long, hipStream_t);
void launch_fused_pair_mask_force_fd(const FusedTable*, int, bool, int, int, int, int, int, unsigned long long, hipStream_t);
void launch_fused_pair_force_x(const FusedTable*, int, bool, int, int, int, int, int, unsigned long long, hipStream_t);
void launch_fused_pair_mask_force_x(const FusedTable*, int, bool, int, int, int, int, int, unsigned long long, hipStream_t);
void launch_fused_pair_force_w(const FusedTable*, int, bool, int, int, int, int, int, unsigned long long, hipStream_t);
void launch_fused_pair_mask_force_w(const FusedTable*, int, bool, int, int, int, int, int, unsigned long long, hipStream_t);
void launch_fused_pair(const FusedTable* dev_table, int metric, bool a_ufirst, bool walls, bool mask, bool force, bool free_drift, int extra,
                       int common, int nstrips, int nchunks, int rows, int write_diag, unsigned long long seq, hipStream_t s) {
    if (metric == 2) walls = true;
    if (extra == 2 && mask) launch_fused_pair_mask_force_w(dev_table, metric, a_ufirst, common, nstrips, nchunks, rows, write_diag, seq, s);
    else if (extra == 2) launch_fused_pair_force_w(dev_table, metric, a_ufirst, common, nstrips, nchunks, rows, write_diag, seq, s);
    else if (extra && mask) launch_fused_pair_mask_force_x(dev_table, metric, a_ufirst, common, nstrips, nchunks, rows, write_diag, seq, s);
    else if (extra) launch_fused_pair_force_x(dev_table, metric, a_ufirst, common, nstrips, nchunks, rows, write_diag, seq, s);
    else if (free_drift && mask) launch_fused_pair_mask_force_fd(dev_table, metric, a_ufirst, common, nstrips, nchunks, rows, write_diag, seq, s);
    else if (free_drift) launch_fused_pair_force_fd(dev_table, metric, a_ufirst, common, nstrips, nchunks, rows, write_diag, seq, s);
    else if (force && mask) launch_fused_pair_mask_force(dev_table, metric, a_ufirst, common, nstrips, nchunks, rows, write_diag, seq, s);
    else if (force) launch_fused_pair_force(dev_table, metric, a_ufirst, common, nstrips, nchunks, rows, write_diag, seq, s);
    else if (mask) launch_fused_pair_mask(dev_table, metric, a_ufirst, common, nstrips, nchunks, rows, write_diag, seq, s);
    else if (walls) launch_fused_pair_walls(dev_table, metric, a_ufirst, common, nstrips, nchunks, rows, write_diag, seq, s);
    else launch_fused_pair_plain(dev_table, metric, a_ufirst, common, nstrips, nchunks, rows, write_diag, seq, s);
}
#endif

}
```

climaseaice.jl_amd/csrc/evp_pair_stage.h:

```cpp
#pragma once
#include "evp_fused_common.h"

namespace csi {
namespace fused {

constexpr int P_LO = 4, P_HI = 59, P_W = P_HI - P_LO + 1;

struct Forcing {
    double t_tau_u, t_we_u, t_wb_u, b_tau_u, b_we_u, b_wb_u, t_tau_v, t_we_v, t_wb_v, b_tau_v, b_we_v, b_wb_v;
    double fd_u, fd_v;
    bool fd;
    double xc_u, xd_u, xc_v, xd_v;
    int extra;
};

struct RowIn { double u_p, v_p, P_0, h_0, a_0, s11, s22, s12, un_m, vn_x; unsigned mk; double ck; };

__device__ __forceinline__ unsigned left_bits(unsigned x) { return (unsigned)__builtin_amdgcn_mov_dpp((int)x, 0x138, 0xf, 0xf, true); }

__device__ __forceinline__ void full_cell(tptr_t T, unsigned o, unsigned s2, double u_0, double v_0, double v_p, double& e11, double& e22, int rcd = 0) {
    const double dyu = c2at(T, C2_DYU + rcd, o), dxv_s = c2at(T, C2_DXV + rcd, o), dxv_n = c2at(T, C2_DXV + rcd, o + s2);
    const double Uy_w = dyu * u_0, Ur_w = fm::rcp(dyu) * u_0;
    const double Vx_s = dxv_s * v_0, Vr_s = fm::rcp(dxv_s) * v_0;
    const double Vx_n = dxv_n * v_p, Vr_n = fm::rcp(dxv_n) * v_p;
    fm::full_strain_cell(from_right(Uy_w), Uy_w, Vx_n, Vx_s, from_right(Ur_w), Ur_w, Vr_n, Vr_s,
                         c2at(T, C2_DYC2 + rcd, o), c2at(T, C2_DXC2 + rcd, o), c2at(T, C2_RAZC + rcd, o), e11, e22);
}
__device__ __forceinline__ double full_corner(tptr_t T, unsigned o, unsigned s2, double u_n, double u_s, double v_e, int rcd = 0) {
    const double Ux_n = c2at(T, C2_RDXU + rcd, o) * u_n, Ux_s = c2at(T, C2_RDXU + rcd, o - s2) * u_s;
    const double Vy_e = c2at(T, C2_RDYV + rcd, o) * v_e;
    return fm::full_strain_corner(Ux_n, Ux_s, Vy_e, from_left(Vy_e), c2at(T, C2_DXF2 + rcd, o), c2at(T, C2_DYF2 + rcd, o), c2at(T, C2_RAZF + rcd, o));
}

template <bool UNI, bool UFIRST, bool MASK, bool TIGHT = false, int CF = 0, bool FULL = false, bool HOLDK = true>
struct Stage {
    double u_m, u_0, v_m, v_0, Xv_m, Xv_0;
    double a_mm, a_m, m_mm, m_m;
    double XP_m, Xm_m, Xa_m, Xe11_m, Xe22_m, Ye12_0, e12_0;
    double XAL_m, XS11L_m, XW, Wprev;
    double XS22L_m;
    double DXV_0, RDXV_0, RDYV_0, RDXU_0, DXF2_0, DYF2_0, RAZF_0;
    double DXV_m, RDXV_m, RDYV_m, RDXU_m, DXF2_m, DYF2_m, DYU_m, RDYU_m, DYC2_m, DXC2_m, DXC2_mm;
    double DXV_p, RDXV_p, RDYV_p, RDXU_p, DXF2_p, DYF2_p, RAZF_p, DYU_0, RDYU_0, DYC2_0, DXC2_0;
#ifndef CSI_FULL_HOISTP
#define CSI_FULL_HOISTP 1
#endif
#if CSI_FULL_HOISTP >= 1
    unsigned long c2p[12];
    int rcd_ = 0;
    __device__ __forceinline__ void hoist_planes(tptr_t T, int rcd = 0) {
        rcd_ = rcd;
#pragma unroll
        for (int k = 0; k < 12; ++k) c2p[k] = T->P[FP_C2_0 + k + rcd];
    }
    __device__ __forceinline__ double c2m(tptr_t, int which, unsigned off) const { return ldg_keep(c2p[which], off); }
#else
    int rcd_ = 0;
    __device__ __forceinline__ void hoist_planes(tptr_t, int rcd = 0) { rcd_ = rcd; }
    __device__ __forceinline__ double c2m(tptr_t T, int which, unsigned off) const { return c2at(T, which + rcd_, off); }
#endif
    __device__ __forceinline__ unsigned long f2u(tptr_t T) const { return T->P[FP_F2U + rcd_]; }
    __device__ __forceinline__ unsigned long f2v(tptr_t T) const { return T->P[FP_F2V + rcd_]; }
    double RAZC_0, RAZU_m, RAZV_x, FU_m, FV_x;

#ifndef CSI_PAIR_VK
#define CSI_PAIR_VK 1
#endif
    static constexpr bool VKC = UNI && !FULL && HOLDK && (CSI_PAIR_VK != 0);
    double VK_E, VK_FN, VK_FS, VK_FU, VK_Q2N, VK_K, VK_FV, VK_BRHO;
    __device__ __forceinline__ void hoist_uniform(tptr_t T) {
        if constexpr (VKC) {
            VK_E = T->K[FK_PCOEF0 + FC_E]; VK_FN = T->K[FK_PCOEF0 + FC_FN]; VK_FS = T->K[FK_PCOEF0 + FC_FS]; VK_FU = T->K[FK_PCOEF0 + FC_FU];
            VK_Q2N = T->K[FK_PCOEF0 + FC_Q2N]; VK_K = T->K[FK_PCOEF0 + FC_K]; VK_FV = T->K[FK_PCOEF0 + FC_FV]; VK_BRHO = T->K[FK_BOT_RHOCD];
            asm volatile("" : "+v"(VK_E), "+v"(VK_FN), "+v"(VK_FS), "+v"(VK_FU), "+v"(VK_Q2N), "+v"(VK_K), "+v"(VK_FV), "+v"(VK_BRHO));
        }
    }
#ifndef CSI_PAIR_LDSC
#define CSI_PAIR_LDSC 0
#endif
    static constexpr bool LDSC = !UNI && !FULL && HOLDK && (CSI_PAIR_LDSC != 0);
    const double* lc = nullptr;
    __device__ __forceinline__ double pc(tptr_t T, int which, int j) const {
        if constexpr (LDSC) return lc[(unsigned)(j & 7) * FC_COUNT + which]; else return pcoef<UNI>(T, which, j);
    }
    __device__ __forceinline__ double vk(tptr_t T, int which, int j, double held) const { if constexpr (VKC) return held; else return pc(T, which, j); }
    __device__ __forceinline__ double brho(tptr_t T) const { if constexpr (VKC) return VK_BRHO; else return T->K[FK_BOT_RHOCD]; }

    double N_DXV, N_RDYV, N_RDXU, N_DXF2, N_DYF2, N_RAZF, N_DYU, N_DYC2, N_DXC2, N_RAZC;
    double N_RAZU, N_RAZV, N_FU, N_FV;
    __device__ __forceinline__ void full_prefetch_vel(tptr_t T, unsigned on, unsigned om) {
        N_RAZU = c2m(T, C2_RAZU, om); N_RAZV = c2m(T, C2_RAZV, UFIRST ? om : on);
        N_FU = 0.0; N_FV = 0.0;
        if (T->I[FI_FKIND] == 2) { N_FU = ldg(f2u(T), om); N_FV = ldg(f2v(T), UFIRST ? om : on); }
    }
    __device__ __forceinline__ void full_prefetch_f(tptr_t T, unsigned on, unsigned om) {
        N_FU = 0.0; N_FV = 0.0;
        if (T->I[FI_FKIND] == 2) { N_FU = ldg(f2u(T), om); N_FV = ldg(f2v(T), UFIRST ? om : on); }
    }
    __device__ __forceinline__ void full_prefetch(tptr_t T, unsigned on, unsigned s2) {
        N_DXV = c2m(T, C2_DXV, on + s2); N_RDYV = c2m(T, C2_RDYV, on + s2); N_RDXU = c2m(T, C2_RDXU, on + s2);
        N_DXF2 = c2m(T, C2_DXF2, on + s2); N_DYF2 = c2m(T, C2_DYF2, on + s2); N_RAZF = c2m(T, C2_RAZF, on + s2);
        N_DYU = c2m(T, C2_DYU, on); N_DYC2 = c2m(T, C2_DYC2, on); N_DXC2 = c2m(T, C2_DXC2, on); N_RAZC = c2m(T, C2_RAZC, on);
    }
    __device__ __forceinline__ void full_init(tptr_t T, unsigned o, unsigned om, unsigned s2) {
        full_prefetch(T, o, s2);
        DXV_0 = c2m(T, C2_DXV, o); RDXV_0 = fm::rcp(DXV_0); RDYV_0 = c2m(T, C2_RDYV, o); RDXU_0 = c2m(T, C2_RDXU, o);
        DXF2_0 = c2m(T, C2_DXF2, o); DYF2_0 = c2m(T, C2_DYF2, o); RAZF_0 = c2m(T, C2_RAZF, o);
        DXV_m = DXV_0; RDXV_m = RDXV_0; RDYV_m = RDYV_0; RDXU_m = RDXU_0; DXF2_m = DXF2_0; DYF2_m = DYF2_0;
        DYU_m = c2m(T, C2_DYU, o); RDYU_m = fm::rcp(DYU_m); DYC2_m = c2m(T, C2_DYC2, o); DXC2_m = c2m(T, C2_DXC2, o); DXC2_mm = DXC2_m;
    }
    double S11_mm, S22_mm, S12_mm, AL_mm, S11_m, S22_m, S12_m, AL_m;
#ifdef CSI_PAIR_PROBE
    unsigned long long sp0 = 0, sp1 = 0, sp2 = 0, sp3 = 0, spt = 0;
#define SPROBE_START do { __builtin_amdgcn_sched_barrier(0); spt = __builtin_readcyclecounter(); __builtin_amdgcn_sched_barrier(0); } while (0)
#define SPROBE(acc) do { __builtin_amdgcn_sched_barrier(0); const unsigned long long t_ = __builtin_readcyclecounter(); \
                         __builtin_amdgcn_sched_barrier(0); acc += t_ - spt; spt = t_; } while (0)
#else
#define SPROBE_START do { } while (0)
#define SPROBE(acc) do { } while (0)
#endif
    double S11_0, S22_0, S12_0, AL_0, zc, zf, Dc, rDc, first, second;
    double Xv_p, Xa_0, Xm_0, e12_p, XW_next;
    double Pf_0, rmc_0, rmf_0;

    struct NoMid { __device__ __forceinline__ void operator()() const {} };
    template <bool PRE = false, class MID = NoMid, bool ALLPRE = false, bool PLR = false>
    __device__ __forceinline__ void step(tptr_t T, const fm::StressConst& ks_in, const fm::VelConst& kv_in, int r,
                                         double u_p, double v_p, double P_0, double m_0, double a_0,
                                         double s11, double s22, double s12, double un_m, double vn_x,
                                         bool do_stress, bool do_vel, bool per_first, bool per_second, unsigned mh,
                                         const Forcing& F, unsigned o2 = 0u, unsigned s2 = 0u, unsigned o2n = 0u, unsigned o2m = 0u, MID mid = MID(), unsigned o2nm = 0u) {
        SPROBE_START;
        Xa_0 = fm::sum2(from_left(a_0), a_0);
        Xv_p = fm::sum2(from_left(v_p), v_p);
        double e11_0, e22_0;
        if constexpr (FULL) {
            DXV_p = N_DXV; RDXV_p = fm::rcp(DXV_p); RDYV_p = N_RDYV; RDXU_p = N_RDXU;
            DXF2_p = N_DXF2; DYF2_p = N_DYF2; RAZF_p = N_RAZF;
            DYU_0 = N_DYU; RDYU_0 = fm::rcp(DYU_0); DYC2_0 = N_DYC2; DXC2_0 = N_DXC2;
            RAZC_0 = N_RAZC;
            if constexpr (ALLPRE) {
                RAZU_m = N_RAZU; RAZV_x = N_RAZV; FU_m = N_FU; FV_x = N_FV;
            } else if (do_vel) {
                RAZU_m = c2m(T, C2_RAZU, o2m); RAZV_x = c2m(T, C2_RAZV, UFIRST ? o2m : o2);
                if (T->I[FI_FKIND] == 2) { FU_m = ldg(f2u(T), o2m); FV_x = ldg(f2v(T), UFIRST ? o2m : o2); }
            }
            const double Uy_w = DYU_0 * u_0, Ur_w = RDYU_0 * u_0;
            fm::full_strain_cell(from_right(Uy_w), Uy_w, DXV_p * v_p, DXV_0 * v_0, from_right(Ur_w), Ur_w, RDXV_p * v_p, RDXV_0 * v_0,
                                 DYC2_0, DXC2_0, RAZC_0, e11_0, e22_0);
            const double Vy_e = RDYV_p * v_p;
            e12_p = fm::full_strain_corner8(RDXU_p * u_p, RDXU_0 * u_0, Vy_e, from_left(Vy_e), DXF2_p, DYF2_p, RAZF_p);
        } else {
        fm::strain_cell<UNI>(pc(T, FC_A, r), pc(T, FC_BN, r), pc(T, FC_BS, r), pc(T, FC_CN, r),
                        pc(T, FC_CS, r), from_right(u_0), u_0, v_p, v_0, e11_0, e22_0);
        e12_p = fm::strain_corner<UNI>(pc(T, FC_SN, r + 1), pc(T, FC_SS, r + 1), pc(T, FC_SV, r + 1),
                                  u_p, u_0, v_p, from_left(v_p));
        }
        {
            const double Xe11_0 = fm::sum2(from_left(e11_0), e11_0), Xe22_0 = fm::sum2(from_left(e22_0), e22_0);
            const double Ye12_p = fm::sum2(e12_p, from_right(e12_p));
            Xm_0 = fm::sum2(from_left(m_0), m_0);
            const double e11f = fm::sum2(Xe11_m, Xe11_0);
            const double e22f = fm::sum2(Xe22_m, Xe22_0);
            const double e12c = 0.0625 * fm::sum2(Ye12_0, Ye12_p);
            const double mf = fm::sum2(Xm_m, Xm_0);
            if constexpr (!PRE) {
                const double XP_0 = fm::sum2(from_left(P_0), P_0);
                Pf_0 = fm::sum2(XP_m, XP_0);
                XP_m = XP_0;
                rmc_0 = fm::rcp(m_0); rmf_0 = fm::rcp(mf);
            }
            const double Pf = Pf_0;
            Xe11_m = Xe11_0; Xe22_m = Xe22_0; Ye12_0 = Ye12_p;
            SPROBE(sp0);
            if (do_stress) {
                fm::StressConst ks = ks_in;
                if (CF) ks.pressure_kind = 0;
                if (TIGHT) {
                    asm volatile("" : "+s"(T));
                    ks.em2 = T->K[FK_EM2]; ks.Dmin = T->K[FK_DMIN]; ks.Dmin2 = T->K[FK_DMIN2]; ks.amin2 = T->K[FK_AMIN2];
                    ks.amax2 = T->K[FK_AMAX2]; ks.hk1 = T->K[FK_HK1]; ks.pressure_kind = T->I[FI_PRESSURE_KIND];
                    ks.em2_8 = T->K[FK_PK_EM2_8]; ks.Dmin2_16 = T->K[FK_PK_DMIN2_16];
                }
                double kc, kf;
                if constexpr (FULL) { kc = T->K[FK_CA_DT] * RAZC_0; kf = T->K[FK_PK_CA_DT4] * RAZF_0; }
                else { kc = UNI ? T->K[FK_HKC] : T->K[FK_CA_DT] * pc(T, FC_RAZC, r); kf = UNI ? T->K[FK_PK_HKF4] : T->K[FK_PK_CA_DT4] * pc(T, FC_RAZF, r); }
                const fm::StressOut o = fm::stress_update_s(ks, e11_0, e22_0, e12_0, e11f, e22f, e12c, P_0, Pf, m_0, mf, rmc_0, rmf_0, kc, kf, s11, s22, s12);
                S11_0 = o.s11; S22_0 = o.s22; S12_0 = o.s12; AL_0 = o.alpha; zc = o.zc2; zf = o.zf2; Dc = o.xc; rDc = o.rDc;
            }
        }
        double d11_0 = S11_0, d22_0 = S22_0, d12_0 = S12_0, d11_m = S11_m, d22_m = S22_m, d12_m = S12_m, d11_mm = S11_mm, d22_mm = S22_mm;
        double d11_mL = XS11L_m, d22_mL = XS22L_m;
        if (MASK) {
            const unsigned m0 = mh & 3u, m1 = (mh >> 2) & 3u, m2 = (mh >> 4) & 3u;
            const bool pcc_0 = m0 == 1u, pcc_m = m1 == 1u, pcc_mm = m2 == 1u;
            unsigned c0 = m0 | m1, c1 = m1 | m2;
            c0 |= left_bits(c0); c1 |= left_bits(c1);
            const bool pff_0 = (c0 & 3u) == 1u, pff_m = (c1 & 3u) == 1u;
            d11_0 = pcc_0 ? 0.0 : S11_0; d22_0 = pcc_0 ? 0.0 : S22_0;
            d11_m = pcc_m ? 0.0 : S11_m; d22_m = pcc_m ? 0.0 : S22_m;
            d11_mm = pcc_mm ? 0.0 : S11_mm; d22_mm = pcc_mm ? 0.0 : S22_mm;
            d12_0 = pff_0 ? 0.0 : S12_0; d12_m = pff_m ? 0.0 : S12_m;
            d11_mL = from_left(d11_m);
            if constexpr (FULL) d22_mL = from_left(d22_m);
            const bool ia_0 = (m0 & 1u) != 0, ia_m = (m1 & 1u) != 0, ia_mm = (m2 & 1u) != 0;
            const bool ia_mL = (left_bits(m1) & 1u) != 0;
            const bool per_u = ia_m | ia_mL;
            per_first = UFIRST ? per_u : (ia_0 | ia_m);
            per_second = UFIRST ? (ia_m | ia_mm) : per_u;
        }
        auto div1_full = [&]() __attribute__((always_inline)) {
            const double S_e = d11_m + d22_m, T_e = DYC2_m * (d11_m - d22_m);
            const double S_w = MASK ? from_left(S_e) : d11_mL + d22_mL;
            const double T_w = MASK ? from_left(T_e) : from_left(DYC2_m) * (d11_mL - d22_mL);
            return fm::full_div1_x2(DYU_m, RDYU_m, RDXU_m, RAZU_m, S_e, S_w, T_e, T_w, DXF2_0 * d12_0, DXF2_m * d12_m);
        };
        auto div2_full = [&](bool low) __attribute__((always_inline)) {
            if (low) {
                const double Zw = DYF2_m * d12_m;
                return fm::full_div2_x2(DXV_m, RDXV_m, RDYV_m, RAZV_x, d11_m + d22_m, d11_mm + d22_mm,
                                     DXC2_m * (d11_m - d22_m), DXC2_mm * (d11_mm - d22_mm), from_right(Zw), Zw);
            }
            const double Zw = DYF2_0 * d12_0;
            return fm::full_div2_x2(DXV_0, RDXV_0, RDYV_0, RAZV_x, d11_0 + d22_0, d11_m + d22_m,
                                 DXC2_0 * (d11_0 - d22_0), DXC2_m * (d11_m - d22_m), from_right(Zw), Zw);
        };
        auto f_full = [&](int which_row, int which_plane, unsigned o, int j) __attribute__((always_inline)) {
            const int kind = T->I[FI_FKIND];
            if (kind == 2) return which_plane == FP_F2U ? FU_m : FV_x;
            if (kind == 1) { typedef const __attribute__((address_space(4))) double* vptr_t; return ((vptr_t)T->P[which_row])[j]; }
            return T->K[FK_FCOR];
        };
        SPROBE(sp1);
        if constexpr (FULL) {
            __builtin_amdgcn_sched_barrier(0);
            if constexpr (!PLR) full_prefetch(T, o2n, s2);
            if constexpr (ALLPRE) { if constexpr (PLR) full_prefetch_f(T, o2n, o2nm); else full_prefetch_vel(T, o2n, o2nm); }
            mid();
            __builtin_amdgcn_sched_barrier(0);
        }
        SPROBE(sp2);
        fm::VelConst kv = kv_in;
        if (TIGHT) {
            asm volatile("" : "+s"(T));
            kv.dt = T->K[FK_DT2]; kv.rdt = T->K[FK_RDT]; kv.min_mass = T->K[FK_MIN_MASS2]; kv.min_conc = T->K[FK_MIN_CONC2];
        }
        if (!do_vel) {
            XW_next = XW;
        } else if (UFIRST) {
            const int j = r - 1;
            double W_0;
            {
                const double vbar = fm::quarter(Xv_m, Xv_0);
                double div;
                if constexpr (FULL) div = div1_full();
                else div = fm::div1(vk(T, FC_E, j, VK_E), vk(T, FC_FN, j, VK_FN), vk(T, FC_FS, j, VK_FS),
                                            d11_m, d11_mL, d12_0, d12_m);
                double ext, imt, exb, imb;
                if (CF) { ext = F.t_tau_u; imt = 0.0; } else fm::ext_stress(T->I[FI_TOP_KIND], F.t_tau_u, T->K[FK_TOP_RHOCD], F.t_we_u, F.t_wb_u, u_m, vbar, ext, imt);
                if (CF == 2) fm::ext_stress_rest(brho(T), u_m, vbar, exb, imb);
                else fm::ext_stress(CF ? 3 : T->I[FI_BOT_KIND], F.b_tau_u, brho(T), F.b_we_u, F.b_wb_u, u_m, vbar, exb, imb);
                double cor;
                if constexpr (FULL) cor = f_full(FP_FROW_U, FP_F2U, o2 - s2, j) * vbar;
                else cor = vk(T, FC_FU, j, VK_FU) * vbar;
                if (F.extra & 1) cor += F.xc_u;
                if (F.extra & 2) div = fm::fma_(2.0, F.xd_u, div);
                W_0 = F.fd ? fm::vel_update_sum_fd(kv, u_m, un_m, Xm_m, Xa_m, XAL_m, div, cor, ext, imt, exb, imb, per_first, F.fd_u)
                           : fm::vel_update_sum(kv, u_m, un_m, Xm_m, Xa_m, XAL_m, div, cor, ext, imt, exb, imb, per_first);
            }
            const double XW_0 = fm::sum2(W_0, from_right(W_0));
            {
                const double ubar = fm::quarter(XW, XW_0);
                double div;
                if constexpr (FULL) div = div2_full(true);
                else div = fm::div2<UNI>(pc(T, FC_Q1N, j), vk(T, FC_Q2N, j, VK_Q2N), pc(T, FC_Q1S, j),
                                            pc(T, FC_Q2S, j), vk(T, FC_K, j, VK_K),
                                            d11_m, d22_m, d11_mm, d22_mm, from_right(d12_m), d12_m);
                double ext, imt, exb, imb;
                if (CF) { ext = F.t_tau_v; imt = 0.0; } else fm::ext_stress(T->I[FI_TOP_KIND], F.t_tau_v, T->K[FK_TOP_RHOCD], F.t_we_v, F.t_wb_v, v_m, ubar, ext, imt);
                if (CF == 2) fm::ext_stress_rest(brho(T), v_m, ubar, exb, imb);
                else fm::ext_stress(CF ? 3 : T->I[FI_BOT_KIND], F.b_tau_v, brho(T), F.b_we_v, F.b_wb_v, v_m, ubar, exb, imb);
                double cor;
                if constexpr (FULL) cor = -f_full(FP_FROW_V, FP_F2V, o2 - s2, j) * ubar;
                else cor = -vk(T, FC_FV, j, VK_FV) * ubar;
                if (F.extra & 1) cor += F.xc_v;
                if (F.extra & 2) div = fm::fma_(2.0, F.xd_v, div);
                second = F.fd ? fm::vel_update_sum_fd(kv, v_m, vn_x, m_mm + m_m, a_mm + a_m, AL_mm + AL_m, div, cor, ext, imt, exb, imb, per_second, F.fd_v)
                              : fm::vel_update_sum(kv, v_m, vn_x, m_mm + m_m, a_mm + a_m, AL_mm + AL_m, div, cor, ext, imt, exb, imb, per_second);
            }
            first = W_0;
            XW_next = XW_0;
        } else {
            double W_0;
            {
                const double ubar = fm::avg4(u_m, from_right(u_m), u_0, from_right(u_0));
                double div;
                if constexpr (FULL) div = div2_full(false);
                else div = fm::div2<UNI>(pc(T, FC_Q1N, r), vk(T, FC_Q2N, r, VK_Q2N), pc(T, FC_Q1S, r),
                                            pc(T, FC_Q2S, r), vk(T, FC_K, r, VK_K),
                                            d11_0, d22_0, d11_m, d22_m, from_right(d12_0), d12_0);
                double ext, imt, exb, imb;
                if (CF) { ext = F.t_tau_v; imt = 0.0; } else fm::ext_stress(T->I[FI_TOP_KIND], F.t_tau_v, T->K[FK_TOP_RHOCD], F.t_we_v, F.t_wb_v, v_0, ubar, ext, imt);
                if (CF == 2) fm::ext_stress_rest(brho(T), v_0, ubar, exb, imb);
                else fm::ext_stress(CF ? 3 : T->I[FI_BOT_KIND], F.b_tau_v, brho(T), F.b_we_v, F.b_wb_v, v_0, ubar, exb, imb);
                double cor;
                if constexpr (FULL) cor = -f_full(FP_FROW_V, FP_F2V, o2, r) * ubar;
                else cor = -vk(T, FC_FV, r, VK_FV) * ubar;
                if (F.extra & 1) cor += F.xc_v;
                if (F.extra & 2) div = fm::fma_(2.0, F.xd_v, div);
                W_0 = F.fd ? fm::vel_update_sum_fd(kv, v_0, vn_x, m_m + m_0, a_m + a_0, AL_m + AL_0, div, cor, ext, imt, exb, imb, per_first, F.fd_v)
                           : fm::vel_update_sum(kv, v_0, vn_x, m_m + m_0, a_m + a_0, AL_m + AL_0, div, cor, ext, imt, exb, imb, per_first);
            }
            const double XW_0 = fm::sum2(from_left(W_0), W_0);
            {
                const int j = r - 1;
                const double vbar = fm::quarter(XW, XW_0);
                double div;
                if constexpr (FULL) div = div1_full();
                else div = fm::div1(vk(T, FC_E, j, VK_E), vk(T, FC_FN, j, VK_FN), vk(T, FC_FS, j, VK_FS),
                                            d11_m, d11_mL, d12_0, d12_m);
                double ext, imt, exb, imb;
                if (CF) { ext = F.t_tau_u; imt = 0.0; } else fm::ext_stress(T->I[FI_TOP_KIND], F.t_tau_u, T->K[FK_TOP_RHOCD], F.t_we_u, F.t_wb_u, u_m, vbar, ext, imt);
                if (CF == 2) fm::ext_stress_rest(brho(T), u_m, vbar, exb, imb);
                else fm::ext_stress(CF ? 3 : T->I[FI_BOT_KIND], F.b_tau_u, brho(T), F.b_we_u, F.b_wb_u, u_m, vbar, exb, imb);
                double cor;
                if constexpr (FULL) cor = f_full(FP_FROW_U, FP_F2U, o2 - s2, j) * vbar;
                else cor = vk(T, FC_FU, j, VK_FU) * vbar;
                if (F.extra & 1) cor += F.xc_u;
                if (F.extra & 2) div = fm::fma_(2.0, F.xd_u, div);
                second = F.fd ? fm::vel_update_sum_fd(kv, u_m, un_m, Xm_m, Xa_m, XAL_m, div, cor, ext, imt, exb, imb, per_second, F.fd_u)
                              : fm::vel_update_sum(kv, u_m, un_m, Xm_m, Xa_m, XAL_m, div, cor, ext, imt, exb, imb, per_second);
            }
            first = W_0;
            XW_next = XW_0;
        }
        SPROBE(sp3);
    }

    __device__ __forceinline__ void shift(double u_p, double v_p, double m_0, double a_0) {
        u_m = u_0; u_0 = u_p; v_m = v_0; v_0 = v_p;
        Xv_m = Xv_0; Xv_0 = Xv_p;
        a_mm = a_m; a_m = a_0; m_mm = m_m; m_m = m_0;
        Xm_m = Xm_0; Xa_m = Xa_0;
        e12_0 = e12_p;
        S11_mm = S11_m; S22_mm = S22_m; S12_mm = S12_m; AL_mm = AL_m;
        S11_m = S11_0; S22_m = S22_0; S12_m = S12_0; AL_m = AL_0;
        XAL_m = fm::sum2(from_left(AL_0), AL_0); XS11L_m = from_left(S11_0);
        if constexpr (FULL) {
            XS22L_m = from_left(S22_0);
            DXV_m = DXV_0; RDXV_m = RDXV_0; RDYV_m = RDYV_0; RDXU_m = RDXU_0; DXF2_m = DXF2_0; DYF2_m = DYF2_0;
            DXV_0 = DXV_p; RDXV_0 = RDXV_p; RDYV_0 = RDYV_p; RDXU_0 = RDXU_p; DXF2_0 = DXF2_p; DYF2_0 = DYF2_p; RAZF_0 = RAZF_p;
            DYU_m = DYU_0; RDYU_m = RDYU_0; DYC2_m = DYC2_0; DXC2_mm = DXC2_m; DXC2_m = DXC2_0;
        }
        XW = XW_next;
        Wprev = first;
    }
};


}
}
```

Baseline: 71.12 billion cell-updates/s.

## Hand over precomputed mass reciprocals and activity predicates from stage A to stage B

Stage A of the paired EVP pipeline now computes the velocity mass reciprocals, area-over-mass ratios and active/positive-mass predicates, and writes them into the shared-memory ring. Stage B reads these instead of recomputing the reciprocals and comparisons from raw mass and area. This removes duplicate rcp and compare work in stage B. In exchange the ring grows by extra LDS fields plus a predicate word array, which adds LDS traffic and footprint. The change also peels the first two B iterations and cuts the final A iteration with matching barriers, to avoid wasted edge-row work.

```diff
diff --git a/climaseaice.jl_amd/csrc/evp_fast_math.h b/climaseaice.jl_amd/csrc/evp_fast_math.h
--- a/climaseaice.jl_amd/csrc/evp_fast_math.h
+++ b/climaseaice.jl_amd/csrc/evp_fast_math.h
@@ -104,10 +104,11 @@
     return o;
 }
 
-__device__ __forceinline__ StressOut stress_update_s(const StressConst& k, double e11c, double e22c, double E12f,
-                                                     double S11f, double S22f, double y2, double Pc, double XP,
-                                                     double mc, double M4, double rmc, double rM4, double hkc, double hkf4,
-                                                     double s11, double s22, double s12) {
+template <bool PRED>
+__device__ __forceinline__ StressOut stress_update_s_(const StressConst& k, double e11c, double e22c, double E12f,
+                                                      double S11f, double S22f, double y2, double Pc, double XP,
+                                                      double mc, double M4, bool mc_pos, bool M4_pos, double rmc, double rM4, double hkc, double hkf4,
+                                                      double s11, double s22, double s12) {
     StressOut o;
     const double dc = e11c + e22c, DF = S11f + S22f;
     const double tc = e11c - e22c, TF = S11f - S22f;
@@ -128,13 +129,25 @@
     double gc, rgc, gf, rgf;
     sqrt_rsqrt(g2c, gc, rgc);
     sqrt_rsqrt(g2f, gf, rgf);
-    const double wc = (mc > 0) ? rgc : 0.0, wf = (M4 > 0) ? rgf : 0.0;
+    const double wc = (PRED ? mc_pos : (mc > 0)) ? rgc : 0.0, wf = (PRED ? M4_pos : (M4 > 0)) ? rgf : 0.0;
     o.s11 = fma_(s11n - s11, wc, s11);
     o.s22 = fma_(s22n - s22, wc, s22);
     o.s12 = fma_(s12n - s12, wf, s12);
     o.alpha = gc;
     o.zc2 = zc2; o.zf2 = zf2; o.xc = xc; o.rDc = rDc;
     return o;
+}
+__device__ __forceinline__ StressOut stress_update_s(const StressConst& k, double e11c, double e22c, double E12f,
+                                                     double S11f, double S22f, double y2, double Pc, double XP,
+                                                     double mc, double M4, double rmc, double rM4, double hkc, double hkf4,
+                                                     double s11, double s22, double s12) {
+    return stress_update_s_<false>(k, e11c, e22c, E12f, S11f, S22f, y2, Pc, XP, mc, M4, false, false, rmc, rM4, hkc, hkf4, s11, s22, s12);
+}
+__device__ __forceinline__ StressOut stress_update_p(const StressConst& k, double e11c, double e22c, double E12f,
+                                                     double S11f, double S22f, double y2, double Pc, double XP,
+                                                     bool mc_pos, bool M4_pos, double rmc, double rM4, double hkc, double hkf4,
+                                                     double s11, double s22, double s12) {
+    return stress_update_s_<true>(k, e11c, e22c, E12f, S11f, S22f, y2, Pc, XP, 0.0, 0.0, mc_pos, M4_pos, rmc, rM4, hkc, hkf4, s11, s22, s12);
 }
 
 __device__ __forceinline__ StressOut stress_update(const StressConst& k, double e11c, double e22c, double e12f,
@@ -199,6 +212,25 @@
     return vel_update_avg_fd(k, w, wn, avg2(m_a, m_b), avg2(a_a, a_b), avg2(al_a, al_b), div, cor, ext, imt, exb, imb, peripheral, wf);
 }
 
+struct VelMass {
+    double rm2, rai;
+    bool active;
+};
+__device__ __forceinline__ VelMass vel_mass(const VelConst& k2, double m2, double a2) {
+    VelMass h;
+    h.rm2 = rcp(m2);
+    h.rai = h.rm2 * a2;
+    h.active = (m2 >= k2.min_mass) & (a2 >= k2.min_conc);
+    return h;
+}
+__device__ __forceinline__ double vel_update_sum_h(const VelConst& k2, double w, double wn, const VelMass& h, double al2,
+                                                   double div2, double cor, double ext, double imt, double exb, double imb, bool peripheral) {
+    const double G = fma_(wn - w, k2.rdt, fma_(div2, h.rm2, fma_(exb - ext, h.rai, cor)));
+    const double tau_i = (imb - imt) * h.rai;
+    const double wD = fma_(k2.dt, G, al2 * w) * rcp(fma_(k2.dt, tau_i, al2));
+    double res = h.active ? wD : 0.0;
+    return peripheral ? 0.0 : res;
+}
 __device__ __forceinline__ double vel_update_sum(const VelConst& k2, double w, double wn, double m2, double a2, double al2,
                                                  double div2, double cor, double ext, double imt, double exb, double imb, bool peripheral) {
     const double rm2 = rcp(m2);
diff --git a/climaseaice.jl_amd/csrc/evp_fused2.hip b/climaseaice.jl_amd/csrc/evp_fused2.hip
--- a/climaseaice.jl_amd/csrc/evp_fused2.hip
+++ b/climaseaice.jl_amd/csrc/evp_fused2.hip
@@ -29,6 +29,15 @@
 #endif
 #ifndef CSI_PAIR_SKIPB
 #define CSI_PAIR_SKIPB 0
+#endif
+#ifndef CSI_PAIR_PEELB
+#define CSI_PAIR_PEELB 1
+#endif
+#ifndef CSI_PAIR_CUTA
+#define CSI_PAIR_CUTA 1
+#endif
+#ifndef CSI_EXP_HANDREG
+#define CSI_EXP_HANDREG 0
 #endif
 #ifndef CSI_PAIR_PD
 #define CSI_PAIR_PD 1
@@ -64,6 +73,10 @@
 #ifndef CSI_PAIR_PRE
 #define CSI_PAIR_PRE 1
 #endif
+#ifndef CSI_PAIR_HAND
+#define CSI_PAIR_HAND 1
+#endif
+enum : int { RF_HU_RM2 = RF_M, RF_HU_RAI = RF_A, RF_HV_RM2 = 13, RF_HV_RAI = 14 };
 #ifndef CSI_PAIR_FRING
 #define CSI_PAIR_FRING 1
 #endif
@@ -80,7 +93,10 @@
     constexpr bool LDSC = !UNI && !FULL && !(EXTRA == 1 && MASK) && (CSI_PAIR_LDSC != 0);
     constexpr bool FRING = FORCE && !FULL && (EXTRA != 1 || !MASK) && CSI_PAIR_FRING;
     constexpr bool PRE = CSI_PAIR_PRE && !MASK && !FULL && !FRING && !(CSI_PAIR_LDSC_NOPRE && !UNI && !(EXTRA == 1 && MASK) && (CSI_PAIR_LDSC != 0));
-    constexpr int RING_FIELDS = FRING ? 10 + RF_FORCING : (PRE ? 13 : 10);
+    constexpr bool HAND = PRE && UNI && !(EXTRA == 1 && MASK) && CSI_PAIR_HAND;
+    static_assert(!HAND || !FD, "the handed-over velocity terms have no free-drift twin (FD comes with FORCE, which has no PRE)");
+    constexpr int RING_FIELDS = FRING ? 10 + RF_FORCING : (HAND ? 15 : (PRE ? 13 : 10));
+    unsigned* const ringw = ringm;
 #define peer_abort (*peer_abort_p)
     const int b = (int)blockIdx.x;
 #ifndef CSI_EXP_ROLESWAP
@@ -479,6 +495,10 @@
         }
 #pragma unroll
         for (int q = 0; q < RING_ROWS * RING_FIELDS; ++q) ring[q * 64 + lane] = 0.0;
+        if constexpr (HAND) {
+#pragma unroll
+            for (int q = 0; q < RING_ROWS; ++q) ringw[q * 64 + lane] = 0u;
+        }
         if constexpr (FULL) {
 #pragma unroll
             for (int q = 0; q < RP_ROWS * RP_FIELDS; ++q) ringp[q * 64 + lane] = 1.0;
@@ -567,7 +587,7 @@
                 A.template step<false>(T, ks, kv, r, C.u_p, C.v_p, C.P_0, m_0, C.a_0, C.s11, C.s22, C.s12, C.un_m, C.vn_x, true, r > rstart, pa1, pa2, mhist, FA,
                                        off2(r), c2s, off2(min(r + 1, rend)), off2(max(r - 1, row0)), mid);
             } else
-            A.step(T, ks, kv, r, C.u_p, C.v_p, C.P_0, m_0, C.a_0, C.s11, C.s22, C.s12, C.un_m, C.vn_x, true, r > rstart, pa1, pa2, mhist, FA);
+            A.template step<false, typename decltype(A)::NoMid, false, false, HAND && !CSI_EXP_HANDREG>(T, ks, kv, r, C.u_p, C.v_p, C.P_0, m_0, C.a_0, C.s11, C.s22, C.s12, C.un_m, C.vn_x, true, r > rstart, pa1, pa2, mhist, FA);
             {
                 const unsigned s0 = rslot(r), s1 = rslot(r - 1);
                 ring[s0 + RF_S11 * 64] = A.S11_0; ring[s0 + RF_S22 * 64] = A.S22_0; ring[s0 + RF_S12 * 64] = A.S12_0;
@@ -576,7 +596,13 @@
                 if (single) {
                     ring[s0 + RF_P * 64] = A.AL_0; ring[s0 + RF_M * 64] = 0.5 * A.zf; ring[s0 + RF_A * 64] = 0.5 * A.zc; ring[s0 + RF_VN * 64] = A.Dc * A.rDc;
                 } else {
-                ring[s0 + RF_P * 64] = C.P_0; ring[s0 + RF_M * 64] = m_0; ring[s0 + RF_A * 64] = C.a_0;
+                ring[s0 + RF_P * 64] = C.P_0;
+                if constexpr (HAND && CSI_EXP_HANDREG) {
+                } else if constexpr (HAND) {
+                    ring[s0 + RF_HU_RM2 * 64] = A.hu_rm2; ring[s0 + RF_HU_RAI * 64] = A.hu_rai;
+                    ring[s0 + RF_HV_RM2 * 64] = A.hv_rm2; ring[s0 + RF_HV_RAI * 64] = A.hv_rai;
+                    ringw[(unsigned)((r - rstart) & (RING_ROWS - 1)) * 64 + lane_it] = A.h_pred;
+                } else { ring[s0 + RF_M * 64] = m_0; ring[s0 + RF_A * 64] = C.a_0; }
                 if (PRE) { ring[s0 + RF_PF * 64] = A.Pf_0; ring[s0 + RF_RMC * 64] = A.rmc_0; ring[s0 + RF_RMF * 64] = A.rmf_0; }
                 ring[s1 + RF_UN * 64] = C.un_m; ring[(AUF ? s1 : s0) + RF_VN * 64] = C.vn_x;
                 }
@@ -622,14 +648,17 @@
             advance();
             load_row(R[1]);
         }
+        const bool cut_last = CSI_PAIR_CUTA && !AUF && !FULL && !single && rend == jb + 3 && rend > rstart;
+        const int rend_a = cut_last ? rend - 1 : rend;
         for (;;) {
             body(Idx<0>{});
-            if (++r > rend) break;
+            if (++r > rend_a) break;
             body(Idx<1>{});
-            if (++r > rend) break;
+            if (++r > rend_a) break;
             body(Idx<2>{});
-            if (++r > rend) break;
-        }
+            if (++r > rend_a) break;
+        }
+        if (cut_last) { __syncthreads(); ++r; }
         for (int d = 0; d < 2; ++d) {
             const unsigned so = (unsigned)((r - rstart) & 1) * (5 * 64) + (unsigned)lane;
             flush(r - 4, outr[so], outr[so + 64], outr[so + 128], outr[so + 192], outr[so + 256], Idx<(7 & ~CSI_PAIR_STORES)>{}, Idx<AUF ? 1 : 0>{});
@@ -701,6 +730,11 @@
     B.S11_mm = 0; B.S22_mm = 0; B.S12_mm = 0; B.AL_mm = 0; B.S11_m = 0; B.S22_m = 0; B.S12_m = 0; B.AL_m = 0;
     B.S11_0 = 0; B.S22_0 = 0; B.S12_0 = 0; B.AL_0 = 0; B.first = 0; B.second = 0;
     B.zc = 0; B.zf = 0; B.Dc = 0; B.rDc = 0; B.Pf_0 = 0; B.rmc_0 = 0; B.rmf_0 = 0;
+    if constexpr (HAND) { B.hu_rm2 = 0; B.hu_rai = 0; B.hv_rm2 = 0; B.hv_rai = 0; B.h_pred = 0; B.Xa_0 = 0; B.Xm_0 = 0; }
+    if constexpr (HAND && CSI_EXP_HANDREG) {
+        B.hu_rm2 = 1e-3; B.hu_rai = 1e-3; B.hv_rm2 = 1e-3; B.hv_rai = 1e-3; B.h_pred = 15u;
+        asm volatile("" : "+v"(B.hu_rm2), "+v"(B.hu_rai), "+v"(B.hv_rm2), "+v"(B.hv_rai), "+v"(B.h_pred));
+    }
     B.hoist_uniform(T);
     if constexpr (FULL) {
         B.hoist_planes(T, rcd);
@@ -715,6 +749,8 @@
     double vn_delay = 0.0;
     double razv_delay = 1.0;
     double fvd_tau = 0.0, fvd_we = 0.0, fvd_wb = 0.0, fvd_fd = 0.0;
+    double hvd_rm2 = 0.0, hvd_rai = 0.0;
+    unsigned hvd_pred = 0u;
     int r = rstart;
     auto bodyB = [&](auto KK) __attribute__((always_inline)) {
         if (!CSI_PAIR_HOIST || FORCE || (FULL && CSI_FULL_FENCE)) asm volatile("" : "+s"(T));
@@ -729,7 +765,24 @@
         const unsigned s1 = rslot(r - 1), s2 = rslot(r - 2), s3 = rslot(r - 3);
         double bu_p = ring[s1 + RF_U * 64], bv_p = ring[s1 + RF_V * 64];
         const double s11 = ring[s2 + RF_S11 * 64], s22 = ring[s2 + RF_S22 * 64], s12 = ring[s2 + RF_S12 * 64];
-        const double bP_0 = ring[s2 + RF_P * 64], bm_0 = ring[s2 + RF_M * 64], ba_0 = ring[s2 + RF_A * 64];
+        const double bP_0 = ring[s2 + RF_P * 64];
+        double bm_0 = 0.0, ba_0 = 0.0;
+        if constexpr (HAND && CSI_EXP_HANDREG) {
+        } else if constexpr (HAND) {
+            typedef decltype(B) SB;
+            B.hu_rm2 = ring[s2 + RF_HU_RM2 * 64]; B.hu_rai = ring[s2 + RF_HU_RAI * 64];
+            const unsigned pw = ringw[(unsigned)((r - 2 - rstart) & (RING_ROWS - 1)) * 64 + lane_it];
+            if (AUF) {
+                B.hv_rm2 = ring[s1 + RF_HV_RM2 * 64]; B.hv_rai = ring[s1 + RF_HV_RAI * 64];
+                const unsigned pv = ringw[(unsigned)((r - 1 - rstart) & (RING_ROWS - 1)) * 64 + lane_it];
+                B.h_pred = (pw & (SB::HP_MC | SB::HP_M4 | SB::HP_U)) | (pv & SB::HP_V);
+            } else {
+                const double n0 = ring[s2 + RF_HV_RM2 * 64], n1 = ring[s2 + RF_HV_RAI * 64];
+                B.hv_rm2 = hvd_rm2; B.hv_rai = hvd_rai;
+                B.h_pred = (pw & (SB::HP_MC | SB::HP_M4 | SB::HP_U)) | hvd_pred;
+                hvd_rm2 = n0; hvd_rai = n1; hvd_pred = pw & SB::HP_V;
+            }
+        } else { bm_0 = ring[s2 + RF_M * 64]; ba_0 = ring[s2 + RF_A * 64]; }
         if (PRE) { B.Pf_0 = ring[s2 + RF_PF * 64]; B.rmc_0 = ring[s2 + RF_RMC * 64]; B.rmf_0 = ring[s2 + RF_RMF * 64]; }
         const double bun = ring[s3 + RF_UN * 64], vn_new = ring[s2 + RF_VN * 64];
         const double bvn = AUF ? vn_new : vn_delay;
@@ -800,7 +853,7 @@
                    off2(max(q, row0)), c2s, off2(max(q + 1, row0)), off2(max(q - 1, row0)), midB, off2(max(q, row0)));
             fq = q; f11 = B.S11_0; f22 = B.S22_0; f12 = B.S12_0; ffirst = B.first; fsecond = B.second; fhave = true;
         } else {
-        B.template step<PRE>(T, ks, kv, q, bu_p, bv_p, bP_0, bm_0, ba_0, s11, s22, s12, bun, bvn, q >= ja - 1, q >= ja, pb1, pb2, mhistB, FB);
+        B.template step<PRE, typename decltype(B)::NoMid, false, false, HAND>(T, ks, kv, q, bu_p, bv_p, bP_0, bm_0, ba_0, s11, s22, s12, bun, bvn, q >= ja - 1, q >= ja, pb1, pb2, mhistB, FB);
         flush(q, B.S11_0, B.S22_0, B.S12_0, B.first, B.second, Idx<(CSI_PAIR_STORES & 7)>{}, Idx<AUF ? 1 : 0>{});
         }
         if ((CSI_PAIR_STORES & 7) != 7) {
@@ -822,6 +875,9 @@
         B.shift(bu_p, bv_p, bm_0, ba_0);
         PROBE(pacc2);
     };
+    if constexpr (!FULL && !MASK && CSI_PAIR_PEELB && !CSI_PAIR_SKIPB) {
+        if (rstart == ja - 3 && rend >= rstart + 2) { __syncthreads(); __syncthreads(); r += 2; }
+    }
     for (;;) {
         bodyB(Idx<0>{});
         if (++r > rend) break;
@@ -847,10 +903,11 @@
                                                               int blocks_per_xcd, int write_diag, unsigned long long seq) {
     constexpr bool FRING = FORCE && !FULL && (EXTRA != 1 || !MASK) && CSI_PAIR_FRING;
     constexpr bool PRE = CSI_PAIR_PRE && !MASK && !FULL && !FRING && !(CSI_PAIR_LDSC_NOPRE && !UNI && !(EXTRA == 1 && MASK) && (CSI_PAIR_LDSC != 0));
-    constexpr int RING_FIELDS = FRING ? 10 + RF_FORCING : (PRE ? 13 : 10);
+    constexpr bool HAND = PRE && UNI && !(EXTRA == 1 && MASK) && CSI_PAIR_HAND;
+    constexpr int RING_FIELDS = FRING ? 10 + RF_FORCING : (HAND ? 15 : (PRE ? 13 : 10));
     __shared__ double ring[RING_ROWS * RING_FIELDS * 64];
     __shared__ double ringp[FULL ? RP_ROWS * RP_FIELDS * 64 : 1];
-    __shared__ unsigned ringm[MASK ? RING_ROWS * 64 : 1];
+    __shared__ unsigned ringm[(MASK || HAND) ? RING_ROWS * 64 : 1];
     __shared__ double outr[(CSI_PAIR_STORES & 7) != 7 ? 2 * 5 * 64 : 1];
     __shared__ unsigned peer_abort_w;
 #ifdef CSI_EXP_LDSPAD
diff --git a/climaseaice.jl_amd/csrc/evp_pair_stage.h b/climaseaice.jl_amd/csrc/evp_pair_stage.h
--- a/climaseaice.jl_amd/csrc/evp_pair_stage.h
+++ b/climaseaice.jl_amd/csrc/evp_pair_stage.h
@@ -122,16 +122,22 @@
     double S11_0, S22_0, S12_0, AL_0, zc, zf, Dc, rDc, first, second;
     double Xv_p, Xa_0, Xm_0, e12_p, XW_next;
     double Pf_0, rmc_0, rmf_0;
-
+    enum : unsigned { HP_MC = 1, HP_M4 = 2, HP_U = 4, HP_V = 8 };
+    double hu_rm2, hu_rai, hv_rm2, hv_rai;
+    unsigned h_pred;
+
+    struct AtU { static constexpr bool value = true; };
+    struct AtV { static constexpr bool value = false; };
     struct NoMid { __device__ __forceinline__ void operator()() const {} };
-    template <bool PRE = false, class MID = NoMid, bool ALLPRE = false, bool PLR = false>
+    template <bool PRE = false, class MID = NoMid, bool ALLPRE = false, bool PLR = false, bool HAND = false>
     __device__ __forceinline__ void step(tptr_t T, const fm::StressConst& ks_in, const fm::VelConst& kv_in, int r,
                                          double u_p, double v_p, double P_0, double m_0, double a_0,
                                          double s11, double s22, double s12, double un_m, double vn_x,
                                          bool do_stress, bool do_vel, bool per_first, bool per_second, unsigned mh,
                                          const Forcing& F, unsigned o2 = 0u, unsigned s2 = 0u, unsigned o2n = 0u, unsigned o2m = 0u, MID mid = MID(), unsigned o2nm = 0u) {
+        constexpr bool TAKE = HAND && PRE, GIVE = HAND && !PRE;
         SPROBE_START;
-        Xa_0 = fm::sum2(from_left(a_0), a_0);
+        if constexpr (!TAKE) Xa_0 = fm::sum2(from_left(a_0), a_0);
         Xv_p = fm::sum2(from_left(v_p), v_p);
         double e11_0, e22_0;
         if constexpr (FULL) {
@@ -159,11 +165,12 @@
         {
             const double Xe11_0 = fm::sum2(from_left(e11_0), e11_0), Xe22_0 = fm::sum2(from_left(e22_0), e22_0);
             const double Ye12_p = fm::sum2(e12_p, from_right(e12_p));
-            Xm_0 = fm::sum2(from_left(m_0), m_0);
+            if constexpr (!TAKE) Xm_0 = fm::sum2(from_left(m_0), m_0);
             const double e11f = fm::sum2(Xe11_m, Xe11_0);
             const double e22f = fm::sum2(Xe22_m, Xe22_0);
             const double e12c = 0.0625 * fm::sum2(Ye12_0, Ye12_p);
-            const double mf = fm::sum2(Xm_m, Xm_0);
+            double mf = 0.0;
+            if constexpr (!TAKE) mf = fm::sum2(Xm_m, Xm_0);
             if constexpr (!PRE) {
                 const double XP_0 = fm::sum2(from_left(P_0), P_0);
                 Pf_0 = fm::sum2(XP_m, XP_0);
@@ -171,6 +178,7 @@
                 rmc_0 = fm::rcp(m_0); rmf_0 = fm::rcp(mf);
             }
             const double Pf = Pf_0;
+            if constexpr (GIVE) h_pred = ((m_0 > 0) ? (unsigned)HP_MC : 0u) | ((mf > 0) ? (unsigned)HP_M4 : 0u);
             Xe11_m = Xe11_0; Xe22_m = Xe22_0; Ye12_0 = Ye12_p;
             SPROBE(sp0);
             if (do_stress) {
@@ -185,7 +193,8 @@
                 double kc, kf;
                 if constexpr (FULL) { kc = T->K[FK_CA_DT] * RAZC_0; kf = T->K[FK_PK_CA_DT4] * RAZF_0; }
                 else { kc = UNI ? T->K[FK_HKC] : T->K[FK_CA_DT] * pc(T, FC_RAZC, r); kf = UNI ? T->K[FK_PK_HKF4] : T->K[FK_PK_CA_DT4] * pc(T, FC_RAZF, r); }
-                const fm::StressOut o = fm::stress_update_s(ks, e11_0, e22_0, e12_0, e11f, e22f, e12c, P_0, Pf, m_0, mf, rmc_0, rmf_0, kc, kf, s11, s22, s12);
+                const fm::StressOut o = TAKE ? fm::stress_update_p(ks, e11_0, e22_0, e12_0, e11f, e22f, e12c, P_0, Pf, (h_pred & HP_MC) != 0, (h_pred & HP_M4) != 0, rmc_0, rmf_0, kc, kf, s11, s22, s12)
+                                             : fm::stress_update_s(ks, e11_0, e22_0, e12_0, e11f, e22f, e12c, P_0, Pf, m_0, mf, rmc_0, rmf_0, kc, kf, s11, s22, s12);
                 S11_0 = o.s11; S22_0 = o.s22; S12_0 = o.s12; AL_0 = o.alpha; zc = o.zc2; zf = o.zf2; Dc = o.xc; rDc = o.rDc;
             }
         }
@@ -245,6 +254,18 @@
             asm volatile("" : "+s"(T));
             kv.dt = T->K[FK_DT2]; kv.rdt = T->K[FK_RDT]; kv.min_mass = T->K[FK_MIN_MASS2]; kv.min_conc = T->K[FK_MIN_CONC2];
         }
+        fm::VelMass hu = {0.0, 0.0, false}, hv = {0.0, 0.0, false};
+        if constexpr (TAKE) {
+            hu.rm2 = hu_rm2; hu.rai = hu_rai; hu.active = (h_pred & HP_U) != 0;
+            hv.rm2 = hv_rm2; hv.rai = hv_rai; hv.active = (h_pred & HP_V) != 0;
+        } else if constexpr (GIVE) {
+            hu = fm::vel_mass(kv, Xm_m, Xa_m);
+            hv = UFIRST ? fm::vel_mass(kv, m_mm + m_m, a_mm + a_m) : fm::vel_mass(kv, m_m + m_0, a_m + a_0);
+        }
+        auto vupd = [&](auto UF, double w, double wn, double al2, double div, double cor,
+                        double ext, double imt, double exb, double imb, bool per) __attribute__((always_inline)) {
+            return fm::vel_update_sum_h(kv, w, wn, decltype(UF)::value ? hu : hv, al2, div, cor, ext, imt, exb, imb, per);
+        };
         if (!do_vel) {
             XW_next = XW;
         } else if (UFIRST) {
@@ -265,6 +286,8 @@
                 else cor = vk(T, FC_FU, j, VK_FU) * vbar;
                 if (F.extra & 1) cor += F.xc_u;
                 if (F.extra & 2) div = fm::fma_(2.0, F.xd_u, div);
+                if constexpr (HAND) W_0 = vupd(AtU{}, u_m, un_m, XAL_m, div, cor, ext, imt, exb, imb, per_first);
+                else
                 W_0 = F.fd ? fm::vel_update_sum_fd(kv, u_m, un_m, Xm_m, Xa_m, XAL_m, div, cor, ext, imt, exb, imb, per_first, F.fd_u)
                            : fm::vel_update_sum(kv, u_m, un_m, Xm_m, Xa_m, XAL_m, div, cor, ext, imt, exb, imb, per_first);
             }
@@ -285,6 +308,8 @@
                 else cor = -vk(T, FC_FV, j, VK_FV) * ubar;
                 if (F.extra & 1) cor += F.xc_v;
                 if (F.extra & 2) div = fm::fma_(2.0, F.xd_v, div);
+                if constexpr (HAND) second = vupd(AtV{}, v_m, vn_x, AL_mm + AL_m, div, cor, ext, imt, exb, imb, per_second);
+                else
                 second = F.fd ? fm::vel_update_sum_fd(kv, v_m, vn_x, m_mm + m_m, a_mm + a_m, AL_mm + AL_m, div, cor, ext, imt, exb, imb, per_second, F.fd_v)
                               : fm::vel_update_sum(kv, v_m, vn_x, m_mm + m_m, a_mm + a_m, AL_mm + AL_m, div, cor, ext, imt, exb, imb, per_second);
             }
@@ -308,6 +333,8 @@
                 else cor = -vk(T, FC_FV, r, VK_FV) * ubar;
                 if (F.extra & 1) cor += F.xc_v;
                 if (F.extra & 2) div = fm::fma_(2.0, F.xd_v, div);
+                if constexpr (HAND) W_0 = vupd(AtV{}, v_0, vn_x, AL_m + AL_0, div, cor, ext, imt, exb, imb, per_first);
+                else
                 W_0 = F.fd ? fm::vel_update_sum_fd(kv, v_0, vn_x, m_m + m_0, a_m + a_0, AL_m + AL_0, div, cor, ext, imt, exb, imb, per_first, F.fd_v)
                            : fm::vel_update_sum(kv, v_0, vn_x, m_m + m_0, a_m + a_0, AL_m + AL_0, div, cor, ext, imt, exb, imb, per_first);
             }
@@ -328,11 +355,17 @@
                 else cor = vk(T, FC_FU, j, VK_FU) * vbar;
                 if (F.extra & 1) cor += F.xc_u;
                 if (F.extra & 2) div = fm::fma_(2.0, F.xd_u, div);
+                if constexpr (HAND) second = vupd(AtU{}, u_m, un_m, XAL_m, div, cor, ext, imt, exb, imb, per_second);
+                else
                 second = F.fd ? fm::vel_update_sum_fd(kv, u_m, un_m, Xm_m, Xa_m, XAL_m, div, cor, ext, imt, exb, imb, per_second, F.fd_u)
                               : fm::vel_update_sum(kv, u_m, un_m, Xm_m, Xa_m, XAL_m, div, cor, ext, imt, exb, imb, per_second);
             }
             first = W_0;
             XW_next = XW_0;
+        }
+        if constexpr (GIVE) {
+            hu_rm2 = hu.rm2; hu_rai = hu.rai; hv_rm2 = hv.rm2; hv_rai = hv.rai;
+            h_pred |= (hu.active ? (unsigned)HP_U : 0u) | (hv.active ? (unsigned)HP_V : 0u);
         }
         SPROBE(sp3);
     }
```

Result: no change. 71.76 billion cell-updates/s, median of 6 (+0.9%).
